# violetdenim/c3dgs

Measured on AMD Instinct MI355X. Metric: raster views/sec fwd+bwd @1920x1080, higher is better.
Workload: dtype f32; 1 GPU; BASELINE.json configs[2]: synth-v1 3M Gaussians, SH deg 3, indexed-camera rasterizer (QAT inner loop), mark_visible+fwd+bwd, 1 view/step/GPU; gaussians=3000000, width=1920, height=1080, sh_codebook=304096, gaussian_codebook=754096, parallelism=replicas x1

## Files before the change

### c3dgs_amd/build.py

```python
import os
import subprocess
import sys
from concurrent.futures import ThreadPoolExecutor

HERE = os.path.dirname(os.path.abspath(__file__))
CSRC = os.path.join(HERE, "csrc")
OBJ = os.path.join(HERE, "build")
LIB = os.path.join(HERE, "libc3dgs_hip.so")
HIPCC = os.environ.get("HIPCC", "/opt/rocm/bin/hipcc")
ARCH = "gfx950"

COMMON = ["--offload-arch=" + ARCH, "-O3", "-fPIC", "-std=c++17", "-Wall", "-Wno-unused-function",
          "-fno-gpu-rdc", "-DNDEBUG"]
SOURCES = {
    "c_abi.hip": [],
    "c_abi_debug.hip": [],
    "preprocess.hip": ["-ffp-contract=off"],
    "backward_preprocess.hip": ["-ffp-contract=off"] + os.environ.get("C3DGS_BWDPRE_FLAGS", "").split(),
    "binning.hip": [],
    "radix_sort.hip": os.environ.get("C3DGS_SORT_FLAGS", "").split(),
    "render.hip": os.environ.get("C3DGS_RENDER_FLAGS", "-fno-slp-vectorize").split(),
    "render_depth.hip": os.environ.get("C3DGS_RENDER_FLAGS", "-fno-slp-vectorize").split(),
    "vq.hip": ["-mllvm", "-amdgpu-mfma-vgpr-form"] + os.environ.get("C3DGS_VQ_FLAGS", "").split(),
    "draws.hip": [],
    "loss.hip": [],
    "metrics.hip": [],
    "encode.hip": [],
    "knn.hip": ["-ffp-contract=off"],
    "adam.hip": ["-ffp-contract=off"],
    "qat.hip": ["-ffp-contract=off"],
    "densify.hip": ["-ffp-contract=off"],
    "index_plan.hip": [],
    "ray_fill.hip": ["-ffp-contract=off"],
    "image_io.hip": ["-ffp-contract=off"],
}
HEADERS = [os.path.join(CSRC, "common.hpp"), os.path.join(CSRC, "gsmath.hpp"), os.path.join(CSRC, "render_diag.hpp"),
           os.path.join(CSRC, "render_common.hpp"),
           os.path.join(HERE, "..", "include", "c3dgs_hip.h"), os.path.join(HERE, "..", "include", "c3dgs_hip_debug.h")]


def _stale(target, deps):
    if not os.path.exists(target):
        return True
    t = os.path.getmtime(target)
    return any(os.path.getmtime(d) > t for d in deps)


def _compile(name, extra, verbose):
    src = os.path.join(CSRC, name)
    obj = os.path.join(OBJ, name.replace(".hip", ".o"))
    cmd = [HIPCC] + COMMON + extra + ["-c", src, "-o", obj]
    if verbose:
        print(" ".join(cmd), flush=True)
    subprocess.check_call(cmd)
    return obj


VARIANTS = {"spin1": {"radix_sort.hip": ["-DC3DGS_OS_SPIN_LIMIT=1u"]}}
def _diag(mode):
    return {src: ["-DC3DGS_DIAG", mode] for src in ("render.hip", "radix_sort.hip", "diag.hip")}


DIAG_VARIANTS = {"lanes": _diag("-DC3DGS_COUNT_LANES"), "bwdtime": _diag("-DC3DGS_BWD_TIMING"), "ostime": _diag("-DC3DGS_OS_TIMING")}


def build_variant(name, verbose=False):
    build(verbose=verbose)
    flags = {**VARIANTS, **DIAG_VARIANTS}[name]
    odir = os.path.join(HERE, "build", "variant_" + name)
    os.makedirs(odir, exist_ok=True)
    lib = os.path.join(HERE, f"libc3dgs_hip_{name}.so")
    objs, rebuilt = [], False
    for src in list(SOURCES) + [f for f in flags if f not in SOURCES]:
        extra = SOURCES.get(src, [])
        obj = os.path.join(OBJ, src.replace(".hip", ".o"))
        if src in flags:
            obj = os.path.join(odir, src.replace(".hip", ".o"))
            if _stale(obj, [os.path.join(CSRC, src)] + HEADERS + [os.path.abspath(__file__)]):
                cmd = [HIPCC] + COMMON + extra + flags[src] + ["-c", os.path.join(CSRC, src), "-o", obj]
                if verbose:
                    print(" ".join(cmd), flush=True)
                subprocess.check_call(cmd)
                rebuilt = True
        objs.append(obj)
    if rebuilt or _stale(lib, objs):
        subprocess.check_call([HIPCC, "--offload-arch=" + ARCH, "-shared", "-fPIC", "-o", lib] + objs)
    return lib


def build(force=False, verbose=False):
    os.makedirs(OBJ, exist_ok=True)
    deps_common = HEADERS + [os.path.abspath(__file__)]
    todo, objs = [], []
    for name, extra in SOURCES.items():
        obj = os.path.join(OBJ, name.replace(".hip", ".o"))
        objs.append(obj)
        if force or _stale(obj, [os.path.join(CSRC, name)] + deps_common):
            todo.append((name, extra))
    if todo:
        with ThreadPoolExecutor(max_workers=min(4, len(todo))) as ex:
            list(ex.map(lambda t: _compile(t[0], t[1], verbose), todo))
    if force or todo or _stale(LIB, objs):
        cmd = [HIPCC, "--offload-arch=" + ARCH, "-shared", "-fPIC", "-o", LIB] + objs
        if verbose:
            print(" ".join(cmd), flush=True)
        subprocess.check_call(cmd)
    return LIB


if __name__ == "__main__":
    print(build(force="--force" in sys.argv, verbose="--verbose" in sys.argv or "-v" in sys.argv))
    for flag, table in (("--variants", VARIANTS), ("--diag", DIAG_VARIANTS)):
        for v in table if flag in sys.argv else ():
            print(build_variant(v, verbose="--verbose" in sys.argv or "-v" in sys.argv))
```

### c3dgs_amd/csrc/binning.hip

```cpp
#include "common.hpp"
#include <rocprim/device/device_radix_sort.hpp>
#include <rocprim/iterator/counting_iterator.hpp>

namespace c3dgs {

size_t scan_temp_bytes(int P)
{
    size_t a = 0, b = 0;
    (void)rocprim::radix_sort_pairs(nullptr, b, (const uint32_t*)nullptr, (uint32_t*)nullptr, (const uint32_t*)nullptr,
                                    (uint32_t*)nullptr, (size_t)P, 0u, 32u);
    size_t m = a > b ? a : b;
    const size_t os = onesweep_depth_temp_bytes(P);
    if (os > m) m = os;
    return m < 256 ? 256 : m;
}

size_t sort_temp_bytes(int R, int end_bit, int key_bytes)
{
    size_t bytes = 0;
    if (key_bytes == 4)
        (void)rocprim::radix_sort_pairs(nullptr, bytes, (const uint32_t*)nullptr, (uint32_t*)nullptr,
                                        (const uint32_t*)nullptr, (uint32_t*)nullptr, (size_t)R, 0u, (unsigned)end_bit);
    else
        (void)rocprim::radix_sort_pairs(nullptr, bytes, (const uint16_t*)nullptr, (uint16_t*)nullptr,
                                        (const uint32_t*)nullptr, (uint32_t*)nullptr, (size_t)R, 0u, (unsigned)end_bit);
    const size_t os = onesweep_tile_temp_bytes(R, end_bit, key_bytes);
    if (os > bytes) bytes = os;
    const size_t reuse = compact_bin_layout(R).bin_bytes;
    if (reuse > bytes) bytes = reuse;
    return bytes < 256 ? 256 : bytes;
}

__global__ void __launch_bounds__(256)
gather_u64_kernel(int n, const uint32_t* __restrict__ idx, const uint2* __restrict__ src, uint2* __restrict__ dst)
{
    const int i = blockIdx.x * 256 + threadIdx.x;
    if (i < n) dst[i] = src[idx[i]];
}

size_t depth_sort_clear_bytes(int P)
{
    return (onesweep_enabled() && (size_t)P < ((size_t)1 << 30)) ? onesweep_depth_clear_bytes(P) : 0;
}
size_t tile_sort_clear_bytes(int R, int end_bit, int key_bytes)
{
    return (onesweep_enabled() && (size_t)R < ((size_t)1 << 30)) ? onesweep_tile_clear_bytes(R, end_bit, key_bytes) : 0;
}

hipError_t run_depth_sort(void* temp, size_t temp_bytes, const uint32_t* kin, uint32_t* kout, const uint32_t* vin,
                          uint32_t* vout, int P, const uint2* rects, uint2* rects_sorted, hipStream_t s, bool ctrl_cleared,
                          bool rects_fit_bytes)
{
    if (onesweep_enabled() && (size_t)P < ((size_t)1 << 30))
        return onesweep_depth_sort(temp, temp_bytes, kin, kout, vin, vout, P, rects, rects_sorted, s, ctrl_cleared, rects_fit_bytes);
    hipError_t e = vin ? rocprim::radix_sort_pairs(temp, temp_bytes, kin, kout, vin, vout, (size_t)P, 0u, 32u, s)
                       : rocprim::radix_sort_pairs(temp, temp_bytes, kin, kout, rocprim::counting_iterator<uint32_t>(0u), vout,
                                                   (size_t)P, 0u, 32u, s);
    if (e != hipSuccess) return e;
    gather_u64_kernel<<<(P + 255) / 256, 256, 0, s>>>(P, vout, rects, rects_sorted);
    return hipGetLastError();
}

hipError_t run_tile_sort(void* temp, size_t temp_bytes, const void* kin, void* kout, int key_bytes, const uint32_t* vin,
                         uint32_t* vout, int R, int end_bit, hipStream_t s, bool ctrl_cleared)
{
    if (key_bytes == 4) {
        if (onesweep_enabled() && (size_t)R < ((size_t)1 << 30))
            return onesweep_tile_sort32(temp, temp_bytes, (const uint32_t*)kin, (uint32_t*)kout, vin, vout, R, end_bit, s, ctrl_cleared);
        return rocprim::radix_sort_pairs(temp, temp_bytes, (const uint32_t*)kin, (uint32_t*)kout, vin, vout, (size_t)R, 0u, (unsigned)end_bit, s);
    }
    if (onesweep_enabled() && (size_t)R < ((size_t)1 << 30))
        return onesweep_tile_sort(temp, temp_bytes, (const uint16_t*)kin, (uint16_t*)kout, vin, vout, R, end_bit, s, ctrl_cleared);
    return rocprim::radix_sort_pairs(temp, temp_bytes, (const uint16_t*)kin, (uint16_t*)kout, vin, vout, (size_t)R, 0u, (unsigned)end_bit, s);
}

}
```

### c3dgs_amd/csrc/c_abi.hip

```cpp
#include "common.hpp"
#include <cfloat>
#include <climits>
#include <cstdlib>
#include <cstring>
#include <mutex>
#include <vector>

namespace c3dgs {

static thread_local std::string g_last_error;
void set_error(const std::string& msg) { g_last_error = msg; }

#define C3DGS_STAGE_TABLE(X)                                                                                                   \
    X(MARK_VISIBLE, "mark_visible") X(PREPROCESS, "preprocess") X(DEPTH_SORT, "depth_sort") X(SCAN, "scan")                    \
    X(DUPLICATE, "duplicate_with_keys") X(SORT, "sort") X(RANGES, "identify_ranges") X(RENDER_FWD, "render_forward")           \
    X(RENDER_DEPTH, "render_depth")                                                                                            \
    X(ZERO_PARTIALS, "zero_partials") X(RENDER_BWD, "render_backward") X(BWD_PREPROCESS, "backward_preprocess")                \
    X(WDIST, "weighted_distance") X(VQ_ACC, "vq_accumulate") X(VQ_APPLY, "vq_apply") X(LOSS_FWD, "l1_ssim_forward")            \
    X(LOSS_BWD, "l1_ssim_backward") X(QAT_OBSERVE, "qat_observe") X(QAT_CODEBOOKS, "qat_codebooks")                            \
    X(QAT_VISIBLE, "qat_visible") X(QAT_POINTS, "qat_points") X(QAT_POINTS_BWD, "qat_points_backward")                         \
    X(QAT_CODEBOOKS_BWD, "qat_codebooks_backward") X(ADAM, "adam_step") X(KNN_SORT, "knn_sort") X(KNN_BOUNDS, "knn_bounds")    \
    X(KNN_QUERY, "knn_query")
#define C3DGS_X(id, name) ST_##id,
enum Stage { C3DGS_STAGE_TABLE(C3DGS_X) ST_COUNT };
#undef C3DGS_X
#define C3DGS_X(id, name) name,
static const char* const kStageNames[ST_COUNT] = { C3DGS_STAGE_TABLE(C3DGS_X) };
#undef C3DGS_X
struct ProfRec { int stage; hipEvent_t a, b; };
static std::mutex g_prof_mu;
static bool g_prof_on = false;
static int g_prof_only = -1;
static std::vector<ProfRec> g_prof_recs;
static std::vector<hipEvent_t> g_prof_pool;

struct StageTimer {
    bool on; int stage; hipStream_t s; hipEvent_t a{}, b{};
    StageTimer(int stage_, hipStream_t s_) : on(g_prof_on && (g_prof_only < 0 || g_prof_only == stage_)), stage(stage_), s(s_)
    {
        if (!on) return;
        std::lock_guard<std::mutex> lk(g_prof_mu);
        auto get = [&](hipEvent_t& e) {
            if (!g_prof_pool.empty()) { e = g_prof_pool.back(); g_prof_pool.pop_back(); }
            else if (hipEventCreate(&e) != hipSuccess) on = false;
        };
        get(a); get(b);
        if (on) (void)hipEventRecord(a, s);
    }
    ~StageTimer()
    {
        if (!on) return;
        (void)hipEventRecord(b, s);
        std::lock_guard<std::mutex> lk(g_prof_mu);
        g_prof_recs.push_back({ stage, a, b });
    }
};
#define C3DGS_STAGE_CHECK(stage, debug, stream) C3DGS_STAGE(kStageNames[stage], debug, stream)
#define C3DGS_TIMED_STAGE(stage, debug, stream, ...)                                                \
    do {                                                                                            \
        { StageTimer t_(stage, stream); __VA_ARGS__; }                                              \
        C3DGS_STAGE_CHECK(stage, debug, stream);                                                    \
    } while (0)

struct HostRead {
    uint32_t* pinned = nullptr;
    uint32_t* dev = nullptr;
    uint32_t seq = 0;
    hipEvent_t ev{};
    HostRead()
    {
        const char* e = std::getenv("C3DGS_HOST_READ_COPY");
        const bool want_map = !(e && e[0] == '1');
        if (want_map && hipHostMalloc((void**)&pinned, 64, hipHostMallocMapped | hipHostMallocPortable | hipHostMallocCoherent) == hipSuccess) {
            void* d = nullptr;
            if (hipHostGetDevicePointer(&d, pinned, 0) == hipSuccess) dev = (uint32_t*)d;
            std::memset(pinned, 0, 64);
        } else {
            (void)hipGetLastError();
            if (hipHostMalloc((void**)&pinned, 64, hipHostMallocDefault) != hipSuccess) { pinned = nullptr; return; }
        }
        if (hipEventCreateWithFlags(&ev, hipEventDisableTiming) != hipSuccess) { (void)hipHostFree(pinned); pinned = nullptr; dev = nullptr; }
    }
    uint32_t begin()
    {
        if (!dev) return 0u;
        if (++seq == 0u) seq = 1u;
        return seq;
    }
    int copy_words(const uint32_t* src, hipStream_t s)
    {
        C3DGS_HIP_TRY(hipMemcpyAsync(pinned, src, 2 * sizeof(uint32_t), hipMemcpyDeviceToHost, s));
        return C3DGS_OK;
    }
    int queue_copy(const uint32_t* src, hipStream_t s)
    {
        if (dev) return C3DGS_OK;
        if (int rc = copy_words(src, s)) return rc;
        C3DGS_HIP_TRY(hipEventRecord(ev, s));
        return C3DGS_OK;
    }
    int wait(const uint32_t* src, hipStream_t s, uint32_t words[2])
    {
        if (dev) {
            volatile uint32_t* pad = pinned;
            bool seen = false;
            for (long spins = 0; !seen; spins++) {
                seen = __atomic_load_n(&pad[2], __ATOMIC_ACQUIRE) == seq;
                if (!seen && (spins & 0xffff) == 0xffff) {
                    const hipError_t q = hipStreamQuery(s);
                    if (q == hipErrorNotReady) continue;
                    if (q != hipSuccess) return fail(C3DGS_E_HIP, std::string("num_rendered read: ") + hipGetErrorString(q));
                    seen = __atomic_load_n(&pad[2], __ATOMIC_ACQUIRE) == seq;
                    if (!seen) {
                        if (int rc = copy_words(src, s)) return rc;
                        C3DGS_HIP_TRY(hipStreamSynchronize(s));
                        seen = true;
                    }
                }
            }
        } else {
            hipError_t q = hipErrorNotReady;
            for (long spins = 0; spins < 20000000L && (q = hipEventQuery(ev)) == hipErrorNotReady; spins++) { }
            if (q == hipErrorNotReady) q = hipEventSynchronize(ev);
            if (q != hipSuccess) return fail(C3DGS_E_HIP, std::string("num_rendered read: ") + hipGetErrorString(q));
        }
        words[0] = pinned[0]; words[1] = pinned[1];
        return C3DGS_OK;
    }
};
static HostRead& host_read()
{
    static thread_local HostRead h;
    return h;
}

static int validate(const c3dgs_raster_params* p, bool indexed, bool is_backward)
{
    if (!p) return fail(C3DGS_E_INVALID, "params is NULL");
    if (p->P < 0 || p->W <= 0 || p->H <= 0) return fail(C3DGS_E_INVALID, "P, W, H must be non-negative / positive");
    if (p->P == 0) return C3DGS_OK;
    if (!p->means3D) return fail(C3DGS_E_INVALID, "means3D must have dimensions (num_points, 3)");
    if (!p->background || !p->viewmatrix || !p->projmatrix || !p->campos)
        return fail(C3DGS_E_INVALID, "background, viewmatrix, projmatrix and campos are required");
    if (!is_backward && !p->opacities)
        return fail(C3DGS_E_INVALID, "opacities is required");
    if ((p->sh == nullptr) == (p->colors_precomp == nullptr))
        return fail(C3DGS_E_INVALID, "Please provide excatly one of either SHs or precomputed colors!");
    const bool has_sr = p->scales != nullptr && p->rotations != nullptr;
    if ((p->scales != nullptr) != (p->rotations != nullptr) || has_sr == (p->cov3D_precomp != nullptr))
        return fail(C3DGS_E_INVALID, "Please provide exactly one of either scale/rotation pair or precomputed 3D covariance!");
    if (p->sh) {
        if (p->D < 0 || p->D > 3) return fail(C3DGS_E_INVALID, "SH degree must be in [0,3]");
        if (p->M < (p->D + 1) * (p->D + 1)) return fail(C3DGS_E_INVALID, "sh has fewer coefficients than the active degree needs");
    }
    if (indexed) {
        if (p->sh && !p->sh_indices) return fail(C3DGS_E_INVALID, "indexed rasterizer: sh_indices is required with sh");
        if (has_sr && (!p->g_indices || !p->scale_factors))
            return fail(C3DGS_E_INVALID, "indexed rasterizer: g_indices and scale_factors are required with scales/rotations");
    } else if (p->sh_indices || p->g_indices || p->scale_factors) {
        return fail(C3DGS_E_INVALID, "non-indexed rasterizer: sh_indices / g_indices / scale_factors must be NULL");
    }
    if (tiles_x(p->W) > 65535 || tiles_y(p->H) > 65535) return fail(C3DGS_E_INVALID, "image too large for 16-bit tile coordinates");
    if ((unsigned long long)tiles_x(p->W) * tiles_x(p->W) * tiles_y(p->H) >= (1ull << 32))
        return fail(C3DGS_E_INVALID, "image too large: (tiles per row)^2 x (tile rows) must stay below 2^32");
    return C3DGS_OK;
}

static int forward_impl(const c3dgs_raster_params* pp, bool indexed, c3dgs_resize_fn geom_resize, void* geom_user,
                        c3dgs_resize_fn binning_resize, void* binning_user, c3dgs_resize_fn image_resize, void* image_user,
                        float* out_color, int32_t* radii, int32_t* num_rendered, void* stream_)
{
    if (int rc = validate(pp, indexed, false)) return rc;
    if (!out_color || !num_rendered) return fail(C3DGS_E_INVALID, "out_color and num_rendered are required");
    if (!geom_resize || !binning_resize || !image_resize) return fail(C3DGS_E_INVALID, "resize callbacks are required");
    c3dgs_raster_params p = *pp;
    if (!indexed) { p.sh_indices = nullptr; p.g_indices = nullptr; p.scale_factors = nullptr; }
    hipStream_t s = (hipStream_t)stream_;
    const int P = p.P, W = p.W, H = p.H;
    const int gx = tiles_x(W), gy = tiles_y(H);
    *num_rendered = 0;

    ImageLayout IL; image_layout(W, H, &IL);
    void* img_base = image_resize(image_user, IL.total_bytes);
    if (!img_base) return fail(C3DGS_E_ALLOC, "image buffer allocation failed");
    const ImgPtrs img = img_ptrs(img_base, W, H);

    if (P == 0) {
        C3DGS_HIP_TRY(hipMemsetAsync(out_color, 0, (size_t)3 * W * H * sizeof(float), s));
        C3DGS_HIP_TRY(hipMemsetAsync(img_base, 0, IL.total_bytes, s));
        return C3DGS_OK;
    }
    if (!radii) return fail(C3DGS_E_INVALID, "radii is required");

    c3dgs_geom_layout GL; geom_layout(P, &GL);
    void* geom_base = geom_resize(geom_user, GL.total_bytes + geom_gtab_bytes(p));
    if (!geom_base) return fail(C3DGS_E_ALLOC, "geometry buffer allocation failed");
    const GeomPtrs g = geom_ptrs(geom_base, P);

    uint32_t* sort_err = onesweep_error_word();
    if (!sort_err) return fail(C3DGS_E_HIP, "cannot resolve the sort error word");
    HostRead& hr = host_read();
    if (!hr.pinned) return fail(C3DGS_E_HIP, "pinned host buffer allocation failed");
    const uint32_t host_seq = hr.begin();
    const size_t dclear = depth_sort_clear_bytes(P) <= g.scan_temp_bytes ? depth_sort_clear_bytes(P) : 0;
    { StageTimer t_(ST_PREPROCESS, s);
      if (geom_gtab_bytes(p)) launch_pack_codebook(p, g.gtab, s);
      launch_preprocess(p, g, radii, img.ranges, sort_err, g.scan_temp, dclear / 16, hr.dev, host_seq, s); }
    C3DGS_STAGE_CHECK(ST_PREPROCESS, p.debug, s);
    const uint32_t* r_words = g.block_base + (P + 255) / 256;
    if (int rc = hr.queue_copy(r_words, s)) return rc;
    { StageTimer t_(ST_DEPTH_SORT, s);
      C3DGS_HIP_TRY(run_depth_sort(g.scan_temp, g.scan_temp_bytes, g.depth_keys, g.depth_keys_sorted, nullptr, g.depth_order, P,
                                   reinterpret_cast<const uint2*>(g.rects), g.sorted_offsets, s, dclear != 0,
                                   gx <= 255 && gy <= 255)); }
    C3DGS_STAGE_CHECK(ST_DEPTH_SORT, p.debug, s);
    if (p.debug && onesweep_timed_out(s)) return fail(C3DGS_E_HIP, "depth sort: look-back timed out");
    C3DGS_TIMED_STAGE(ST_SCAN, p.debug, s, launch_depth_order_scan(P, g, s));
    uint32_t words[2];
    if (int rc = hr.wait(r_words, s, words)) return rc;
    const uint32_t R_u = words[0];
    if (words[1] != 0) {
        C3DGS_HIP_TRY(hipMemsetAsync(sort_err, 0, sizeof(uint32_t), s));
        return fail(C3DGS_E_HIP, "radix sort look-back timed out in an earlier rasterizer call on this device: that call's "
                                 "image is NaN and its gradients are invalid (flag cleared, this call was not run)");
    }
    if (R_u > 0x7fffffffu) return fail(C3DGS_E_INVALID, "num_rendered overflows int32");
    const int R = (int)R_u;
    *num_rendered = R;

    c3dgs_binning_layout BL; binning_layout(R, W, H, &BL);
    void* bin_base = binning_resize(binning_user, BL.total_bytes);
    if (!bin_base) return fail(C3DGS_E_ALLOC, "binning buffer allocation failed");
    const BinPtrs b = bin_ptrs(bin_base, R, W, H);

    if (R > 0) {
        const int end_bit = tile_sort_end_bit(W, H);
        size_t tclear = tile_sort_clear_bytes(R, end_bit, b.key_bytes);
        if (tclear > b.sort_temp_bytes) tclear = 0;
        C3DGS_TIMED_STAGE(ST_DUPLICATE, p.debug, s, launch_duplicate_with_keys(P, g, b, gx, sort_err, b.sort_temp, tclear / 16, s));
        { StageTimer t_(ST_SORT, s);
          C3DGS_HIP_TRY(run_tile_sort(b.sort_temp, b.sort_temp_bytes, b.keys_unsorted, b.keys_sorted, b.key_bytes, b.values_unsorted,
                                      b.point_list, R, end_bit, s, tclear != 0)); }
        C3DGS_STAGE_CHECK(ST_SORT, p.debug, s);
        if (p.debug && onesweep_timed_out(s)) return fail(C3DGS_E_HIP, "tile sort: look-back timed out");
        C3DGS_TIMED_STAGE(ST_RANGES, p.debug, s, launch_identify_ranges(R, b.keys_sorted, b.key_bytes, img.ranges, sort_err, s));
    }
    C3DGS_TIMED_STAGE(ST_RENDER_FWD, p.debug, s,
                      launch_render_forward(W, H, img, b.point_list, g.splat, p.background, out_color, compact_ptrs(b, R), sort_err, s));
    return C3DGS_OK;
}

static int backward_impl(const c3dgs_raster_params* pp, bool indexed, const int32_t* radii, const void* geom_buffer,
                         const void* binning_buffer, const void* image_buffer, int32_t R, const float* dL_dout_color,
                         c3dgs_resize_fn ws_resize, void* ws_user, const c3dgs_raster_grads* grads, void* stream_)
{
    if (int rc = validate(pp, indexed, true)) return rc;
    if (!grads) return fail(C3DGS_E_INVALID, "grads is NULL");
    c3dgs_raster_params p = *pp;
    if (!indexed) { p.sh_indices = nullptr; p.g_indices = nullptr; p.scale_factors = nullptr; }
    hipStream_t s = (hipStream_t)stream_;
    const int P = p.P, W = p.W, H = p.H;

    void* cb_zero = nullptr;
    size_t cb_zero16 = 0;
    if (indexed) {
        const size_t n_sh = (grads->dL_dsh && p.sh) ? (size_t)p.SHS * p.M * 3 * sizeof(float) : 0;
        const size_t n_rot = (grads->dL_drotations && p.scales) ? (size_t)p.GS * 4 * sizeof(float) : 0;
        const size_t n_sc = (grads->dL_dscales && p.scales) ? (size_t)p.GS * 3 * sizeof(float) : 0;
        char* a_sh = (char*)grads->dL_dsh; char* a_rot = (char*)grads->dL_drotations; char* a_sc = (char*)grads->dL_dscales;
        if (n_sh && n_rot && n_sc && a_rot == a_sh + n_sh && a_sc == a_rot + n_rot) {
            const size_t n = n_sh + n_rot + n_sc;
            if (p.P > 0 && R >= 0 && ((uintptr_t)a_sh & 15u) == 0) {
                cb_zero = a_sh; cb_zero16 = n / 16;
                if (n % 16) C3DGS_HIP_TRY(hipMemsetAsync(a_sh + cb_zero16 * 16, 0, n % 16, s));
            } else {
                C3DGS_HIP_TRY(hipMemsetAsync(a_sh, 0, n, s));
            }
        } else {
            if (n_sh) C3DGS_HIP_TRY(hipMemsetAsync(a_sh, 0, n_sh, s));
            if (n_sc) C3DGS_HIP_TRY(hipMemsetAsync(a_sc, 0, n_sc, s));
            if (n_rot) C3DGS_HIP_TRY(hipMemsetAsync(a_rot, 0, n_rot, s));
        }
    }
    if (P == 0) return C3DGS_OK;
    if (!radii || !geom_buffer || !image_buffer || !dL_dout_color || (R > 0 && !binning_buffer))
        return fail(C3DGS_E_INVALID, "radii, forward buffers and dL_dout_color are required");
    if (!ws_resize) return fail(C3DGS_E_INVALID, "workspace callback is required");
    if (R < 0) return fail(C3DGS_E_INVALID, "R must be >= 0");

    const GeomPtrs g = geom_ptrs(const_cast<void*>(geom_buffer), P);
    const ImgPtrs img = img_ptrs(const_cast<void*>(image_buffer), W, H);
    void* ws_base = ws_resize(ws_user, c3dgs_backward_workspace_bytes(P, R));
    if (!ws_base) return fail(C3DGS_E_ALLOC, "backward workspace allocation failed");
    const BwdPtrs w = bwd_ptrs(ws_base, P, R);

    { StageTimer t_(ST_ZERO_PARTIALS, s);
      launch_backward_prep(R > 0 ? W : 0, H, img, w.touched, w.touched_bytes / 16, R > 0 ? nullptr : cb_zero, R > 0 ? 0 : cb_zero16, s); }
    if (R > 0) {
        const BinPtrs b = bin_ptrs(const_cast<void*>(binning_buffer), R, W, H);
        C3DGS_TIMED_STAGE(ST_RENDER_BWD, p.debug, s,
                          launch_render_backward(W, H, img, g.splat, g.block_base, p.background, dL_dout_color, w.partials, w.touched,
                                                 compact_ptrs(b, R), cb_zero, cb_zero16, s));
    }
    C3DGS_TIMED_STAGE(ST_BWD_PREPROCESS, p.debug, s, launch_backward_preprocess(p, radii, g, w, *grads, s));
    return C3DGS_OK;
}

}

using namespace c3dgs;

extern "C" {

const char* c3dgs_last_error(void) { return g_last_error.c_str(); }

int c3dgs_profile_enable(int on)
{
    std::lock_guard<std::mutex> lk(g_prof_mu);
    g_prof_on = on != 0;
    return C3DGS_OK;
}

int c3dgs_profile_only(const char* stage_name)
{
    std::lock_guard<std::mutex> lk(g_prof_mu);
    g_prof_only = -1;
    if (!stage_name || !*stage_name) return C3DGS_OK;
    for (int i = 0; i < ST_COUNT; i++)
        if (std::strcmp(stage_name, kStageNames[i]) == 0) { g_prof_only = i; return C3DGS_OK; }
    return fail(C3DGS_E_INVALID, std::string("profile_only: unknown stage ") + stage_name);
}

int c3dgs_profile_read(c3dgs_stage_time* out, int capacity)
{
    std::vector<ProfRec> recs;
    {
        std::lock_guard<std::mutex> lk(g_prof_mu);
        recs.swap(g_prof_recs);
    }
    double total[ST_COUNT] = { 0 };
    long long count[ST_COUNT] = { 0 };
    for (auto& r : recs) {
        float ms = 0.f;
        if (hipEventSynchronize(r.b) == hipSuccess && hipEventElapsedTime(&ms, r.a, r.b) == hipSuccess) {
            total[r.stage] += (double)ms;
            count[r.stage]++;
        }
    }
    {
        std::lock_guard<std::mutex> lk(g_prof_mu);
        for (auto& r : recs) { g_prof_pool.push_back(r.a); g_prof_pool.push_back(r.b); }
    }
    int n = 0;
    for (int i = 0; i < ST_COUNT && n < capacity; i++) {
        if (!count[i]) continue;
        std::memset(&out[n], 0, sizeof(out[n]));
        std::strncpy(out[n].name, kStageNames[i], sizeof(out[n].name) - 1);
        out[n].total_ms = total[i];
        out[n].count = count[i];
        n++;
    }
    return n;
}
int c3dgs_abi_version(void) { return C3DGS_ABI_VERSION; }

int c3dgs_get_geom_layout(int32_t P, c3dgs_geom_layout* out)
{
    if (!out || P < 0) return fail(C3DGS_E_INVALID, "bad arguments");
    geom_layout(P, out);
    return C3DGS_OK;
}
int c3dgs_get_binning_layout(int32_t R, int32_t W, int32_t H, c3dgs_binning_layout* out)
{
    if (!out || R < 0 || W <= 0 || H <= 0) return fail(C3DGS_E_INVALID, "bad arguments");
    binning_layout(R, W, H, out);
    return C3DGS_OK;
}
int c3dgs_get_image_layout(int32_t W, int32_t H, c3dgs_image_layout* out)
{
    if (!out || W <= 0 || H <= 0) return fail(C3DGS_E_INVALID, "bad arguments");
    ImageLayout L; image_layout(W, H, &L);
    *out = L;
    return C3DGS_OK;
}
int c3dgs_get_compact_layout(int32_t R, int32_t W, int32_t H, c3dgs_compact_layout* out)
{
    if (!out || R < 0 || W <= 0 || H <= 0) return fail(C3DGS_E_INVALID, "bad arguments");
    c3dgs_binning_layout BL; binning_layout(R, W, H, &BL);
    const CompactBinLayout C = compact_bin_layout(R);
    ImageLayout IL; image_layout(W, H, &IL);
    out->cqm = BL.sort_temp + C.cqm; out->cid = BL.sort_temp + C.cid;
    out->tile_used_c = IL.tile_used_c; out->n_contrib_c = IL.n_contrib_c;
    return C3DGS_OK;
}
int c3dgs_get_backward_layout(int32_t P, int32_t R, c3dgs_backward_layout* out)
{
    if (!out || P < 0 || R < 0) return fail(C3DGS_E_INVALID, "bad arguments");
    backward_layout(P, R, out);
    return C3DGS_OK;
}
size_t c3dgs_backward_workspace_bytes(int32_t P, int32_t R)
{
    c3dgs_backward_layout L; backward_layout(P, R, &L);
    return L.total_bytes;
}

int c3dgs_mark_visible(int32_t P, const float* means3D, const float* viewmatrix, const float* projmatrix, uint8_t* present,
                       void* stream)
{
    (void)projmatrix;
    if (P < 0) return fail(C3DGS_E_INVALID, "P must be >= 0");
    if (P == 0) return C3DGS_OK;
    if (!means3D || !viewmatrix || !present) return fail(C3DGS_E_INVALID, "means3D, viewmatrix and present are required");
    C3DGS_TIMED_STAGE(ST_MARK_VISIBLE, 0, (hipStream_t)stream, launch_mark_visible(P, means3D, viewmatrix, present, (hipStream_t)stream));
    return C3DGS_OK;
}

int c3dgs_mark_visible_pose(int32_t P, const float* means3D, const float* extrinsic_vector, uint8_t* present, void* stream)
{
    if (P < 0) return fail(C3DGS_E_INVALID, "P must be >= 0");
    if (P == 0) return C3DGS_OK;
    if (!means3D || !extrinsic_vector || !present) return fail(C3DGS_E_INVALID, "means3D, extrinsic_vector and present are required");
    C3DGS_TIMED_STAGE(ST_MARK_VISIBLE, 0, (hipStream_t)stream, launch_mark_visible_pose(P, means3D, extrinsic_vector, present, (hipStream_t)stream));
    return C3DGS_OK;
}

int c3dgs_camera_from_pose(const float* extrinsic_vector, float inv_tan_half_fovx, float inv_tan_half_fovy, float* viewmatrix,
                           float* projmatrix, float* campos, void* stream)
{
    if (!extrinsic_vector || !viewmatrix || !projmatrix || !campos) return fail(C3DGS_E_INVALID, "camera_from_pose: NULL pointer");
    launch_camera_from_pose(extrinsic_vector, inv_tan_half_fovx, inv_tan_half_fovy, viewmatrix, projmatrix, campos, (hipStream_t)stream);
    C3DGS_STAGE("camera_from_pose", 0, (hipStream_t)stream);
    return C3DGS_OK;
}

int c3dgs_rasterize_gaussians(const c3dgs_raster_params* p, c3dgs_resize_fn geom_resize, void* geom_user,
                              c3dgs_resize_fn binning_resize, void* binning_user, c3dgs_resize_fn image_resize,
                              void* image_user, float* out_color, int32_t* radii, int32_t* num_rendered, void* stream)
{
    return forward_impl(p, false, geom_resize, geom_user, binning_resize, binning_user, image_resize, image_user, out_color,
                        radii, num_rendered, stream);
}

int c3dgs_rasterize_gaussians_indexed(const c3dgs_raster_params* p, c3dgs_resize_fn geom_resize, void* geom_user,
                                      c3dgs_resize_fn binning_resize, void* binning_user, c3dgs_resize_fn image_resize,
                                      void* image_user, float* out_color, int32_t* radii, int32_t* num_rendered, void* stream)
{
    return forward_impl(p, true, geom_resize, geom_user, binning_resize, binning_user, image_resize, image_user, out_color,
                        radii, num_rendered, stream);
}

int c3dgs_rasterize_gaussians_backward(const c3dgs_raster_params* p, const int32_t* radii, const void* geom_buffer,
                                       const void* binning_buffer, const void* image_buffer, int32_t R,
                                       const float* dL_dout_color, c3dgs_resize_fn workspace_resize, void* workspace_user,
                                       const c3dgs_raster_grads* grads, void* stream)
{
    return backward_impl(p, false, radii, geom_buffer, binning_buffer, image_buffer, R, dL_dout_color, workspace_resize,
                         workspace_user, grads, stream);
}

int c3dgs_rasterize_gaussians_backward_indexed(const c3dgs_raster_params* p, const int32_t* radii, const void* geom_buffer,
                                               const void* binning_buffer, const void* image_buffer, int32_t R,
                                               const float* dL_dout_color, c3dgs_resize_fn workspace_resize,
                                               void* workspace_user, const c3dgs_raster_grads* grads, void* stream)
{
    return backward_impl(p, true, radii, geom_buffer, binning_buffer, image_buffer, R, dL_dout_color, workspace_resize,
                         workspace_user, grads, stream);
}

int c3dgs_render_depth(int32_t P, int32_t W, int32_t H, int32_t R, const void* geom_buffer, const void* binning_buffer,
                       const void* image_buffer, float* out_depth, float* out_alpha, float* out_median, void* stream)
{
    if (W <= 0 || H <= 0) return fail(C3DGS_E_INVALID, "render_depth: W and H must be positive");
    if (P < 0 || R < 0) return fail(C3DGS_E_INVALID, "render_depth: P and R must be >= 0");
    if (!out_depth && !out_alpha && !out_median) return fail(C3DGS_E_INVALID, "render_depth: at least one output is required");
    if (R > 0 && P == 0) return fail(C3DGS_E_INVALID, "render_depth: R > 0 instances cannot come from P = 0");
    if (R > 0 && (!geom_buffer || !binning_buffer || !image_buffer))
        return fail(C3DGS_E_INVALID, "render_depth: the forward's geometry, binning and image buffers are required");
    hipStream_t s = (hipStream_t)stream;
    if (P == 0 || R == 0) {
        const size_t bytes = (size_t)W * H * sizeof(float);
        for (float* o : { out_depth, out_alpha, out_median })
            if (o) C3DGS_HIP_TRY(hipMemsetAsync(o, 0, bytes, s));
        return C3DGS_OK;
    }
    uint32_t* sort_err = onesweep_error_word();
    if (!sort_err) return fail(C3DGS_E_HIP, "cannot resolve the sort error word");
    const GeomPtrs g = geom_ptrs(const_cast<void*>(geom_buffer), P);
    const ImgPtrs img = img_ptrs(const_cast<void*>(image_buffer), W, H);
    const BinPtrs b = bin_ptrs(const_cast<void*>(binning_buffer), R, W, H);
    C3DGS_TIMED_STAGE(ST_RENDER_DEPTH, 0, s,
                      launch_render_depth(W, H, img, compact_ptrs(b, R), g.splat, g.depth_keys, out_depth, out_alpha, out_median,
                                          sort_err, s));
    return C3DGS_OK;
}

int c3dgs_weighted_distance(int64_t N, int32_t C, int32_t K, const float* coefs, const int64_t* gather,
                            const float* codebook, float* out_dist, int64_t* out_idx, void* stream)
{
    if (N < 0 || C < 0 || K <= 0) return fail(C3DGS_E_INVALID, "coefs and codebook must have same number of channels");
    if (N == 0) return C3DGS_OK;
    if (!coefs || !codebook || !out_dist || !out_idx) return fail(C3DGS_E_INVALID, "ceofs and codebook must have dimension 2");
    {
        StageTimer t_(ST_WDIST, (hipStream_t)stream);
        if (launch_weighted_distance(N, C, K, coefs, gather, codebook, out_dist, out_idx, (hipStream_t)stream))
            return fail(C3DGS_E_INVALID, "unsupported channel count");
    }
    C3DGS_STAGE_CHECK(ST_WDIST, 0, (hipStream_t)stream);
    return C3DGS_OK;
}

size_t c3dgs_weighted_distance_ws_bytes(int64_t N, int32_t C, int32_t K) { return wd_ws_bytes(N, C, K); }

int c3dgs_weighted_distance_ws(int64_t N, int32_t C, int32_t K, const float* coefs, const int64_t* gather, const float* codebook,
                               float* out_dist, int64_t* out_idx, void* ws, size_t ws_bytes, void* stream)
{
    if (N < 0 || C < 0 || K <= 0) return fail(C3DGS_E_INVALID, "coefs and codebook must have same number of channels");
    if (N == 0) return C3DGS_OK;
    if (!coefs || !codebook || !out_dist || !out_idx) return fail(C3DGS_E_INVALID, "ceofs and codebook must have dimension 2");
    {
        StageTimer t_(ST_WDIST, (hipStream_t)stream);
        if (launch_weighted_distance(N, C, K, coefs, gather, codebook, out_dist, out_idx, (hipStream_t)stream, ws, ws ? ws_bytes : 0))
            return fail(C3DGS_E_INVALID, "unsupported channel count");
    }
    C3DGS_STAGE_CHECK(ST_WDIST, 0, (hipStream_t)stream);
    return C3DGS_OK;
}

int c3dgs_vq_accumulate(int64_t B, int32_t K, int32_t D, const float* x, const float* w, const int64_t* gather,
                        const int64_t* idx, const float* dist, float* S, double* dist_sum, void* stream)
{
    if (B < 0 || K <= 0 || D <= 0) return fail(C3DGS_E_INVALID, "bad sizes");
    if (B == 0) return C3DGS_OK;
    if (!x || !w || !idx || !S) return fail(C3DGS_E_INVALID, "x, w, idx and S are required");
    C3DGS_TIMED_STAGE(ST_VQ_ACC, 0, (hipStream_t)stream, launch_vq_accumulate(B, K, D, x, w, gather, idx, dist, S, dist_sum, (hipStream_t)stream));
    return C3DGS_OK;
}

int c3dgs_vq_sums(int64_t B, int32_t K, int32_t D, const float* x, const float* w, const int64_t* gather,
                  const float* codebook, float* dist, int64_t* idx, float* S, double* dist_sum, void* ws, size_t ws_bytes,
                  void* stream)
{
    if (B < 0 || K <= 0 || D <= 0) return fail(C3DGS_E_INVALID, "bad sizes");
    if (!S || !dist_sum) return fail(C3DGS_E_INVALID, "S and dist_sum are required");
    C3DGS_HIP_TRY(hipMemsetAsync(S, 0, (size_t)K * (D + 1) * sizeof(float), (hipStream_t)stream));
    C3DGS_HIP_TRY(hipMemsetAsync(dist_sum, 0, sizeof(double), (hipStream_t)stream));
    if (B == 0) return C3DGS_OK;
    if (!x || !w || !codebook || !dist || !idx) return fail(C3DGS_E_INVALID, "x, w, codebook, dist and idx are required");
    {
        StageTimer t_(ST_WDIST, (hipStream_t)stream);
        if (launch_weighted_distance(B, K, D, x, gather, codebook, dist, idx, (hipStream_t)stream, ws, ws ? ws_bytes : 0))
            return fail(C3DGS_E_INVALID, "unsupported channel count");
    }
    C3DGS_STAGE_CHECK(ST_WDIST, 0, (hipStream_t)stream);
    return c3dgs_vq_accumulate(B, K, D, x, w, gather, idx, dist, S, dist_sum, stream);
}

int c3dgs_vq_step_supported(int32_t K, int32_t D, const float* x, const float* codebook, const void* ws, size_t ws_bytes)
{
    return (K > 0 && D > 0 && wd_presplit_supported(K, D, x, codebook, ws, ws_bytes)) ? 1 : 0;
}

int c3dgs_vq_step_sums(int32_t step, int64_t B, int32_t K, int32_t D, const float* x, const float* w, const int64_t* gather,
                       const float* codebook, float* dist, int64_t* idx, float* S, double* dist_sum, void* ws, size_t ws_bytes,
                       void* stream)
{
    hipStream_t s = (hipStream_t)stream;
    if (step < 0 || B <= 0 || K <= 0 || D <= 0) return fail(C3DGS_E_INVALID, "vq_step_sums: bad sizes");
    if (!x || !w || !codebook || !dist || !idx || !S || !dist_sum) return fail(C3DGS_E_INVALID, "vq_step_sums: NULL argument");
    if (!wd_presplit_supported(K, D, x, codebook, ws, ws_bytes))
        return fail(C3DGS_E_INVALID, "vq_step_sums: shape / scratch not served by the fused step (see c3dgs_vq_step_supported)");
    if (step == 0) {
        C3DGS_HIP_TRY(hipMemsetAsync(S, 0, (size_t)K * (D + 1) * sizeof(float), s));
        C3DGS_HIP_TRY(hipMemsetAsync(dist_sum, 0, sizeof(double), s));
    }
    {
        StageTimer t_(ST_WDIST, s);
        if (launch_weighted_distance(B, K, D, x, gather, codebook, dist, idx, s, ws, ws_bytes, step == 0 ? -1 : (step & 1)))
            return fail(C3DGS_E_INVALID, "vq_step_sums: unsupported shape");
        if (step == 0) launch_vq_seed_words(K, D, ws, s);
    }
    C3DGS_STAGE_CHECK(ST_WDIST, 0, s);
    C3DGS_TIMED_STAGE(ST_VQ_ACC, 0, s,
                      launch_vq_accumulate(B, K, D, x, w, gather, idx, dist, S, dist_sum, s, vq_next_absmax_word(K, D, ws, step & 1)));
    return C3DGS_OK;
}

int c3dgs_vq_step_apply(int32_t step, int32_t K, int32_t D, float* S, float* codebook, float* entry_importance, float decay,
                        float alpha, float eps, int32_t scale_normalize, void* ws, size_t ws_bytes, void* stream)
{
    if (step < 0 || K <= 0 || D <= 0 || !S || !codebook || !entry_importance) return fail(C3DGS_E_INVALID, "vq_step_apply: bad arguments");
    { StageTimer t_(ST_VQ_APPLY, (hipStream_t)stream);
      if (launch_vq_apply_split(K, D, S, codebook, entry_importance, decay, alpha, eps, scale_normalize, ws, ws_bytes, step & 1, (hipStream_t)stream))
          return fail(C3DGS_E_INVALID, "vq_step_apply: shape / scratch not served by the fused step (see c3dgs_vq_step_supported)"); }
    C3DGS_STAGE_CHECK(ST_VQ_APPLY, 0, (hipStream_t)stream);
    return C3DGS_OK;
}

int c3dgs_vq_apply(int32_t K, int32_t D, const float* S, float* codebook, float* entry_importance, float decay,
                   float alpha, float eps, int32_t scale_normalize, void* stream)
{
    if (K <= 0 || D <= 0 || !S || !codebook || !entry_importance) return fail(C3DGS_E_INVALID, "bad arguments");
    C3DGS_TIMED_STAGE(ST_VQ_APPLY, 0, (hipStream_t)stream,
                      launch_vq_apply(K, D, S, codebook, entry_importance, decay, alpha, eps, scale_normalize, (hipStream_t)stream));
    return C3DGS_OK;
}

size_t c3dgs_morton_workspace_bytes(int32_t P) { return morton_workspace_bytes(P); }

int c3dgs_morton_order(int32_t P, const float* xyz, int64_t* codes, int64_t* order, void* workspace, void* stream)
{
    if (P < 0) return fail(C3DGS_E_INVALID, "P must be >= 0");
    if (P == 0) return C3DGS_OK;
    if (!xyz || !codes || !order || !workspace) return fail(C3DGS_E_INVALID, "morton_order: bad arguments");
    if (run_morton_order(P, xyz, codes, order, workspace, (hipStream_t)stream)) return fail(C3DGS_E_HIP, "morton_order failed");
    C3DGS_STAGE("morton_order", 0, (hipStream_t)stream);
    return C3DGS_OK;
}

size_t c3dgs_knn_workspace_bytes(int32_t P) { return knn_workspace_bytes(P); }

int c3dgs_knn_mean_dist2(int32_t P, const float* xyz, float* out, void* workspace, void* stream)
{
    if (P < 0) return fail(C3DGS_E_INVALID, "knn_mean_dist2: P must be >= 0");
    if (P == 0) return C3DGS_OK;
    if (!xyz || !out || !workspace) return fail(C3DGS_E_INVALID, "knn_mean_dist2: bad arguments");
    hipStream_t s = (hipStream_t)stream;
    { StageTimer t_(ST_KNN_SORT, s);
      if (run_knn_sort(P, xyz, workspace, s)) return fail(C3DGS_E_HIP, "knn_mean_dist2: sort failed"); }
    C3DGS_STAGE_CHECK(ST_KNN_SORT, 0, s);
    C3DGS_TIMED_STAGE(ST_KNN_BOUNDS, 0, s, launch_knn_bounds(P, workspace, s));
    C3DGS_TIMED_STAGE(ST_KNN_QUERY, 0, s, launch_knn_query(P, workspace, out, s));
    return C3DGS_OK;
}

int c3dgs_knn_neighbours(int32_t P, const float* xyz, int32_t* idx, float* d2, void* workspace, void* stream)
{
    if (P < 0) return fail(C3DGS_E_INVALID, "knn_neighbours: P must be >= 0");
    if (P == 0) return C3DGS_OK;
    if (!xyz || !idx || !d2 || !workspace) return fail(C3DGS_E_INVALID, "knn_neighbours: bad arguments");
    hipStream_t s = (hipStream_t)stream;
    { StageTimer t_(ST_KNN_SORT, s);
      if (run_knn_sort(P, xyz, workspace, s)) return fail(C3DGS_E_HIP, "knn_neighbours: sort failed"); }
    C3DGS_STAGE_CHECK(ST_KNN_SORT, 0, s);
    C3DGS_TIMED_STAGE(ST_KNN_BOUNDS, 0, s, launch_knn_bounds(P, workspace, s));
    C3DGS_TIMED_STAGE(ST_KNN_QUERY, 0, s, launch_knn_query_neighbours(P, workspace, idx, d2, s));
    return C3DGS_OK;
}

int c3dgs_abs_accumulate(int64_t n, const float* g, float* acc, void* stream)
{
    if (n < 0 || (n > 0 && (!g || !acc))) return fail(C3DGS_E_INVALID, "abs_accumulate: bad arguments");
    launch_abs_accumulate(n, g, acc, (hipStream_t)stream);
    C3DGS_STAGE("abs_accumulate", 0, (hipStream_t)stream);
    return C3DGS_OK;
}

int c3dgs_adam_step(int32_t n_tensors, const c3dgs_adam_tensor* tensors, double beta1, double beta2, double eps, void* stream)
{
    if (n_tensors < 0 || n_tensors > C3DGS_ADAM_MAX_TENSORS) return fail(C3DGS_E_INVALID, "adam_step: between 0 and 16 tensors per call");
    if (n_tensors == 0) return C3DGS_OK;
    if (!tensors) return fail(C3DGS_E_INVALID, "adam_step: tensors is NULL");
    for (int k = 0; k < n_tensors; k++)
        if (tensors[k].n > 0 && (!tensors[k].param || !tensors[k].grad || !tensors[k].exp_avg || !tensors[k].exp_avg_sq))
            return fail(C3DGS_E_INVALID, "adam_step: NULL tensor pointer");
    C3DGS_TIMED_STAGE(ST_ADAM, 0, (hipStream_t)stream, launch_adam(n_tensors, tensors, beta1, beta2, eps, (hipStream_t)stream));
    return C3DGS_OK;
}

static const int kRowsMaxCopies = 250;

int c3dgs_densify_classify(int32_t P, const float* accum, const float* denom, const float* scale_clone, const float* scale_split,
                           const float* scale_prune_self, const float* scale_prune_child, const float* opacity, float max_grad,
                           float dense_extent, float min_opacity, float big_extent, uint8_t* code, void* stream)
{
    if (P < 0) return fail(C3DGS_E_INVALID, "densify_classify: P must be >= 0");
    if (!(max_grad > 0.f)) return fail(C3DGS_E_INVALID, "densify_classify: max_grad must be > 0 (see include/c3dgs_hip.h)");
    if (P == 0) return C3DGS_OK;
    if (!accum || !denom || !scale_clone || !scale_split || !opacity || !code)
        return fail(C3DGS_E_INVALID, "densify_classify: NULL buffer");
    if ((scale_prune_self == nullptr) != (scale_prune_child == nullptr))
        return fail(C3DGS_E_INVALID, "densify_classify: scale_prune_self and scale_prune_child go together");
    launch_densify_classify(P, accum, denom, scale_clone, scale_split, scale_prune_self, scale_prune_child, opacity, max_grad,
                            dense_extent, min_opacity, big_extent, code, (hipStream_t)stream);
    C3DGS_STAGE("densify_classify", 0, (hipStream_t)stream);
    return C3DGS_OK;
}

size_t c3dgs_rows_plan_workspace_bytes(int32_t P) { return rows_plan_workspace_bytes(P); }

int c3dgs_rows_plan(int32_t P, const uint8_t* code, int32_t N, int64_t capacity, int32_t* src, uint8_t* kind, int32_t* draw_row,
                    int32_t* totals, void* workspace, void* stream)
{
    if (P < 0) return fail(C3DGS_E_INVALID, "rows_plan: P must be >= 0");
    if (N < 1 || N > kRowsMaxCopies) return fail(C3DGS_E_INVALID, "rows_plan: N must be between 1 and 250");
    if (capacity < 0) return fail(C3DGS_E_INVALID, "rows_plan: capacity must be >= 0");
    if ((int64_t)P * (2 + N) >= ((int64_t)1 << 31)) return fail(C3DGS_E_INVALID, "rows_plan: P * (2 + N) must fit 31 bits");
    if (!totals) return fail(C3DGS_E_INVALID, "rows_plan: totals is required");
    hipStream_t s = (hipStream_t)stream;
    if (P == 0) { C3DGS_HIP_TRY(hipMemsetAsync(totals, 0, 4 * sizeof(int32_t), s)); return C3DGS_OK; }
    if (!code || !workspace) return fail(C3DGS_E_INVALID, "rows_plan: NULL buffer");
    if (src && (!kind || !draw_row)) return fail(C3DGS_E_INVALID, "rows_plan: src, kind and draw_row go together");
    C3DGS_HIP_TRY(run_rows_plan(P, code, N, capacity, src, kind, draw_row, totals, workspace, s));
    C3DGS_STAGE("rows_plan", 0, s);
    return C3DGS_OK;
}

int c3dgs_rows_apply(int32_t P, int64_t P_new, const int32_t* src, const uint8_t* kind, const int32_t* draw_row, int32_t n_tensors,
                     const c3dgs_rows_tensor* tensors, int32_t N, int64_t n_draws, const float* rotation_raw, const float* std,
                     const float* z, int32_t log_scaling, int32_t half_xyz, void* stream)
{
    if (P < 0 || P_new < 0 || n_draws < 0) return fail(C3DGS_E_INVALID, "rows_apply: sizes must be >= 0");
    if (N < 1 || N > kRowsMaxCopies) return fail(C3DGS_E_INVALID, "rows_apply: N must be between 1 and 250");
    if (n_tensors < 0 || n_tensors > C3DGS_ROWS_MAX_TENSORS) return fail(C3DGS_E_INVALID, "rows_apply: between 0 and 16 tensors per call");
    if (P_new >= ((int64_t)1 << 31)) return fail(C3DGS_E_INVALID, "rows_apply: P_new must fit 31 bits");
    if (P_new == 0 || n_tensors == 0) return C3DGS_OK;
    if (P == 0) return fail(C3DGS_E_INVALID, "rows_apply: P_new > 0 rows cannot come from P = 0");
    if (!src || !kind || !draw_row || !tensors) return fail(C3DGS_E_INVALID, "rows_apply: NULL buffer");
    for (int k = 0; k < n_tensors; k++) {
        const c3dgs_rows_tensor& t = tensors[k];
        if (t.row_floats < 1 || t.row_floats > 4096) return fail(C3DGS_E_INVALID, "rows_apply: row_floats must be between 1 and 4096");
        if (!t.in_param || !t.out_param) return fail(C3DGS_E_INVALID, "rows_apply: NULL tensor pointer");
        const int nm = (t.in_exp_avg != nullptr) + (t.in_exp_avg_sq != nullptr) + (t.out_exp_avg != nullptr) + (t.out_exp_avg_sq != nullptr);
        if (nm != 0 && nm != 4) return fail(C3DGS_E_INVALID, "rows_apply: the four moment pointers go together");
        if (t.role != C3DGS_ROLE_COPY && t.role != C3DGS_ROLE_XYZ && t.role != C3DGS_ROLE_SCALING)
            return fail(C3DGS_E_INVALID, "rows_apply: unknown role");
        if (t.role != C3DGS_ROLE_COPY && t.row_floats != 3) return fail(C3DGS_E_INVALID, "rows_apply: xyz / scaling rows have 3 floats");
        if (t.role != C3DGS_ROLE_COPY && n_draws > 0 && (!std || !z || (t.role == C3DGS_ROLE_XYZ && !rotation_raw)))
            return fail(C3DGS_E_INVALID, "rows_apply: children need rotation_raw, std and z");
    }
    launch_rows_apply(P, P_new, src, kind, draw_row, n_tensors, tensors, N, n_draws, rotation_raw, std, z, log_scaling, half_xyz, (hipStream_t)stream);
    C3DGS_STAGE("rows_apply", 0, (hipStream_t)stream);
    return C3DGS_OK;
}

int c3dgs_densify_stats(int32_t P, const float* grad, const uint8_t* filter, const int32_t* radii, float* accum, float* denom,
                        float* max_radii, void* stream)
{
    if (P < 0) return fail(C3DGS_E_INVALID, "densify_stats: P must be >= 0");
    if (P == 0) return C3DGS_OK;
    if (!grad || !filter || !accum || !denom) return fail(C3DGS_E_INVALID, "densify_stats: NULL buffer");
    if ((radii == nullptr) != (max_radii == nullptr)) return fail(C3DGS_E_INVALID, "densify_stats: radii and max_radii go together");
    launch_densify_stats(P, grad, filter, radii, accum, denom, max_radii, (hipStream_t)stream);
    C3DGS_STAGE("densify_stats", 0, (hipStream_t)stream);
    return C3DGS_OK;
}

size_t c3dgs_ray_fill_plan_workspace_bytes(int32_t P, int64_t rows) { return ray_fill_plan_workspace_bytes(P, rows); }

int c3dgs_ray_fill_plan(int32_t P, const float* d2, float step, int64_t capacity, int32_t* src, uint8_t* slot, int32_t* level,
                        int32_t* totals, void* workspace, size_t workspace_bytes, void* stream)
{
    if (P < 0 || capacity < 0) return fail(C3DGS_E_INVALID, "ray_fill_plan: P and capacity must be >= 0");
    if (P > INT32_MAX - 255) return fail(C3DGS_E_INVALID, "ray_fill_plan: P must be at most INT32_MAX - 255");
    if (!(step > 0.f) || !(step <= FLT_MAX)) return fail(C3DGS_E_INVALID, "ray_fill_plan: step must be a positive finite number");
    if (!totals) return fail(C3DGS_E_INVALID, "ray_fill_plan: totals is required");
    if (src && (!slot || !level)) return fail(C3DGS_E_INVALID, "ray_fill_plan: src, slot and level go together");
    hipStream_t s = (hipStream_t)stream;
    if (P == 0) { C3DGS_HIP_TRY(hipMemsetAsync(totals, 0, 4 * sizeof(int32_t), s)); return C3DGS_OK; }
    if (!d2 || !workspace) return fail(C3DGS_E_INVALID, "ray_fill_plan: NULL buffer");
    std::string problem;
    C3DGS_HIP_TRY(run_ray_fill_plan(P, d2, step, capacity, src, slot, level, totals, workspace, workspace_bytes, s, &problem));
    if (!problem.empty()) return fail(C3DGS_E_INVALID, "ray_fill_plan: " + problem);
    C3DGS_STAGE("ray_fill_plan", 0, s);
    return C3DGS_OK;
}

int c3dgs_ray_fill_xyz(int32_t P, const float* xyz, const int32_t* idx, const float* d2, float step, int64_t n_new,
                       const int32_t* src, const uint8_t* slot, const int32_t* level, float* out, void* stream)
{
    if (P < 0 || n_new < 0) return fail(C3DGS_E_INVALID, "ray_fill_xyz: sizes must be >= 0");
    if (n_new > INT32_MAX - 255) return fail(C3DGS_E_INVALID, "ray_fill_xyz: n_new must be at most INT32_MAX - 255");
    if (!(step > 0.f) || !(step <= FLT_MAX)) return fail(C3DGS_E_INVALID, "ray_fill_xyz: step must be a positive finite number");
    if (n_new == 0) return C3DGS_OK;
    if (!xyz || !idx || !d2 || !src || !slot || !level || !out) return fail(C3DGS_E_INVALID, "ray_fill_xyz: NULL buffer");
    launch_ray_fill_xyz(P, xyz, idx, d2, step, n_new, src, slot, level, out, (hipStream_t)stream);
    C3DGS_STAGE("ray_fill_xyz", 0, (hipStream_t)stream);
    return C3DGS_OK;
}

int c3dgs_image_from_u8(int32_t Hs, int32_t Ws, int32_t C, const uint8_t* src, int32_t flip, const float* bg, int32_t Hd, int32_t Wd,
                        float* out, void* stream)
{
    const int32_t kMax = 32768;
    if (Hs < 1 || Ws < 1 || Hd < 1 || Wd < 1 || Hs > kMax || Ws > kMax || Hd > kMax || Wd > kMax)
        return fail(C3DGS_E_INVALID, "image_from_u8: every dimension must be in [1, 32768]");
    if (C != 3 && C != 4) return fail(C3DGS_E_INVALID, "image_from_u8: C must be 3 or 4");
    if (bg && C == 3) return fail(C3DGS_E_INVALID, "image_from_u8: a background needs an alpha channel (C == 4)");
    if (!src || !out) return fail(C3DGS_E_INVALID, "image_from_u8: NULL buffer");
    launch_image_from_u8(Hs, Ws, C, src, flip != 0, bg, Hd, Wd, out, (hipStream_t)stream);
    C3DGS_STAGE("image_from_u8", 0, (hipStream_t)stream);
    return C3DGS_OK;
}

static const int32_t kIndexPlanMaxRows = INT32_MAX - 255;

size_t c3dgs_index_plan_workspace_bytes(int32_t P, int32_t K0, int32_t K1) { return index_plan_workspace_bytes(P, K0, K1); }

int c3dgs_index_plan(int32_t P, const uint8_t* keep, const int64_t* idx0, int32_t K0, const int64_t* idx1, int32_t K1, int64_t cap_rows,
                     int64_t cap_cb0, int64_t cap_cb1, int32_t* src, int64_t* new_idx0, int64_t* new_idx1, int32_t* cb_src0,
                     int32_t* cb_src1, int32_t* totals, void* workspace, void* stream)
{
    if (P < 0 || K0 < 0 || K1 < 0) return fail(C3DGS_E_INVALID, "index_plan: P, K0 and K1 must be >= 0");
    if (P > kIndexPlanMaxRows || K0 > kIndexPlanMaxRows || K1 > kIndexPlanMaxRows)
        return fail(C3DGS_E_INVALID, "index_plan: P, K0 and K1 must be at most INT32_MAX - 255");
    if (cap_rows < 0 || cap_cb0 < 0 || cap_cb1 < 0) return fail(C3DGS_E_INVALID, "index_plan: capacities must be >= 0");
    if ((idx0 && K0 <= 0) || (idx1 && K1 <= 0)) return fail(C3DGS_E_INVALID, "index_plan: an index array needs a codebook of K > 0 rows");
    if (!totals) return fail(C3DGS_E_INVALID, "index_plan: totals is required");
    if (!workspace) return fail(C3DGS_E_INVALID, "index_plan: workspace is required");
    if (src && ((idx0 && (!new_idx0 || !cb_src0)) || (idx1 && (!new_idx1 || !cb_src1))))
        return fail(C3DGS_E_INVALID, "index_plan: src, and new_idx and cb_src of every index space given, go together");
    hipStream_t s = (hipStream_t)stream;
    if (P == 0) { C3DGS_HIP_TRY(hipMemsetAsync(totals, 0, 4 * sizeof(int32_t), s)); return C3DGS_OK; }
    C3DGS_HIP_TRY(run_index_plan(P, keep, idx0, K0, idx1, K1, cap_rows, cap_cb0, cap_cb1, src, new_idx0, new_idx1, cb_src0, cb_src1,
                                 totals, workspace, s));
    C3DGS_STAGE("index_plan", 0, s);
    return C3DGS_OK;
}

int c3dgs_extract_rot_scale(int32_t n, const float* cov6, float* rot, float* scale, void* stream)
{
    if (n < 0) return fail(C3DGS_E_INVALID, "extract_rot_scale: n must be >= 0");
    if (n == 0) return C3DGS_OK;
    if (!cov6 || !rot || !scale || (reinterpret_cast<uintptr_t>(rot) & 15)) return fail(C3DGS_E_INVALID, "extract_rot_scale: bad arguments");
    launch_extract_rot_scale(n, cov6, rot, scale, (hipStream_t)stream);
    C3DGS_STAGE("extract_rot_scale", 0, (hipStream_t)stream);
    return C3DGS_OK;
}

int c3dgs_l1_ssim_forward(int32_t C, int32_t H, int32_t W, const float* img, const float* gt, float* dmaps, double* sums,
                          void* stream)
{
    if (C <= 0 || H <= 0 || W <= 0 || !img || !gt || !sums) return fail(C3DGS_E_INVALID, "l1_ssim_forward: bad arguments");
    hipStream_t s = (hipStream_t)stream;
    C3DGS_HIP_TRY(hipMemsetAsync(sums, 0, 128 * sizeof(double), s));
    const size_t n = (size_t)C * H * W;
    C3DGS_TIMED_STAGE(ST_LOSS_FWD, 0, s,
                      launch_l1_ssim_forward(C, H, W, img, gt, dmaps, dmaps ? dmaps + n : nullptr, dmaps ? dmaps + 2 * n : nullptr, sums, s));
    return C3DGS_OK;
}

int c3dgs_l1_ssim_value(const double* sums, double l1_scale, double ssim_scale, double constant, float* out, void* stream)
{
    if (!sums || !out) return fail(C3DGS_E_INVALID, "l1_ssim_value: bad arguments");
    launch_l1_ssim_value(sums, l1_scale, ssim_scale, constant, out, (hipStream_t)stream);
    C3DGS_STAGE("l1_ssim_value", 0, (hipStream_t)stream);
    return C3DGS_OK;
}

int c3dgs_l1_ssim_backward(int32_t C, int32_t H, int32_t W, const float* img, const float* gt, const float* dmaps,
                           const float* grad_loss, float l1_coeff, float ssim_coeff, float* dL_dimg, void* stream)
{
    if (C <= 0 || H <= 0 || W <= 0 || !img || !gt || !dmaps || !grad_loss || !dL_dimg)
        return fail(C3DGS_E_INVALID, "l1_ssim_backward: bad arguments");
    hipStream_t s = (hipStream_t)stream;
    const size_t n = (size_t)C * H * W;
    C3DGS_TIMED_STAGE(ST_LOSS_BWD, 0, s,
                      launch_l1_ssim_backward(C, H, W, img, gt, dmaps, dmaps + n, dmaps + 2 * n, grad_loss, l1_coeff, ssim_coeff, dL_dimg, s));
    return C3DGS_OK;
}

size_t c3dgs_image_metrics_ws_bytes(int32_t N, int32_t C, int32_t H, int32_t W) { return image_metrics_ws_bytes(N, C, H, W); }

int c3dgs_image_metrics(int32_t N, int32_t C, int32_t H, int32_t W, const float* img, const float* gt, void* ws, size_t ws_bytes,
                        double* out, void* stream)
{
    if (N <= 0 || C <= 0 || H <= 0 || W <= 0) return fail(C3DGS_E_INVALID, "image_metrics: N, C, H and W must be positive");
    if (image_metrics_workgroups(N, C, H, W) > IMAGE_METRICS_MAX_WORKGROUPS)
        return fail(C3DGS_E_INVALID, "image_metrics: size overflow (N * C * H * W too large for one call; split the batch)");
    if (!img || !gt || !ws || !out) return fail(C3DGS_E_INVALID, "image_metrics: img, gt, ws and out are required");
    if (reinterpret_cast<uintptr_t>(ws) & 7) return fail(C3DGS_E_INVALID, "image_metrics: ws must be 8-byte aligned");
    const size_t need = image_metrics_ws_bytes(N, C, H, W);
    if (ws_bytes < need)
        return fail(C3DGS_E_INVALID, "image_metrics: ws too small (" + std::to_string(ws_bytes) + " bytes, need " +
                                         std::to_string(need) + ")");
    launch_image_metrics(N, C, H, W, img, gt, (double*)ws, out, (hipStream_t)stream);
    C3DGS_STAGE("image_metrics", 0, (hipStream_t)stream);
    return C3DGS_OK;
}

static int qat_validate(const c3dgs_qat_params* q, const char* who)
{
    if (!q) return fail(C3DGS_E_INVALID, std::string(who) + ": params is NULL");
    if (q->P < 0 || q->GS < 0 || q->SHS < 0 || q->M < 1) return fail(C3DGS_E_INVALID, std::string(who) + ": bad sizes");
    if (!q->state) return fail(C3DGS_E_INVALID, std::string(who) + ": state is required");
    if (q->features_dc && q->M > 1 && !q->features_rest)
        return fail(C3DGS_E_INVALID, std::string(who) + ": features_rest is required with features_dc when M > 1");
    if (reinterpret_cast<uintptr_t>(q->rotation) & 15) return fail(C3DGS_E_INVALID, std::string(who) + ": rotation must be 16-byte aligned");
    return C3DGS_OK;
}
static bool misaligned16(const void* p) { return (reinterpret_cast<uintptr_t>(p) & 15) != 0; }

size_t c3dgs_qat_workspace_bytes(void) { return qat_workspace_bytes(); }
size_t c3dgs_qat_scan_bytes(int32_t P) { return qat_scan_bytes(P); }

int c3dgs_qat_observe(const c3dgs_qat_params* q, void* workspace, void* stream)
{
    if (int rc = qat_validate(q, "qat_observe")) return rc;
    if (!workspace) return fail(C3DGS_E_INVALID, "qat_observe: workspace is required");
    C3DGS_TIMED_STAGE(ST_QAT_OBSERVE, 0, (hipStream_t)stream, launch_qat_observe(*q, workspace, (hipStream_t)stream));
    return C3DGS_OK;
}

int c3dgs_qat_codebooks(const c3dgs_qat_params* q, float* scales_n, float* rotations, float* shs, void* stream)
{
    if (int rc = qat_validate(q, "qat_codebooks")) return rc;
    if (misaligned16(rotations) || misaligned16(shs)) return fail(C3DGS_E_INVALID, "qat_codebooks: outputs must be 16-byte aligned");
    C3DGS_TIMED_STAGE(ST_QAT_CODEBOOKS, 0, (hipStream_t)stream, launch_qat_codebooks(*q, scales_n, rotations, shs, (hipStream_t)stream));
    return C3DGS_OK;
}

int c3dgs_qat_codebooks_backward(const c3dgs_qat_params* q, const float* dL_dscales_n, const float* dL_drotations,
                                 const float* dL_dshs, float* dL_dscaling, float* dL_drotation, float* dL_dfeatures_dc,
                                 float* dL_dfeatures_rest, void* stream)
{
    if (int rc = qat_validate(q, "qat_codebooks_backward")) return rc;
    if (misaligned16(dL_drotations) || misaligned16(dL_drotation) || misaligned16(dL_dshs))
        return fail(C3DGS_E_INVALID, "qat_codebooks_backward: rotation / sh gradients must be 16-byte aligned");
    if (dL_dshs && q->features_dc && (!dL_dfeatures_dc || (q->M > 1 && !dL_dfeatures_rest)))
        return fail(C3DGS_E_INVALID, "qat_codebooks_backward: dL_dfeatures_dc / dL_dfeatures_rest are required with dL_dshs");
    C3DGS_TIMED_STAGE(ST_QAT_CODEBOOKS_BWD, 0, (hipStream_t)stream,
                      launch_qat_codebooks_backward(*q, dL_dscales_n, dL_drotations, dL_dshs, dL_dscaling, dL_drotation, dL_dfeatures_dc,
                                                    dL_dfeatures_rest, (hipStream_t)stream));
    return C3DGS_OK;
}

int c3dgs_qat_visible(const c3dgs_qat_params* q, const float* viewmatrix, uint8_t* visible, int32_t* rank, int32_t* count,
                      void* scan_workspace, void* stream)
{
    if (int rc = qat_validate(q, "qat_visible")) return rc;
    if (!count) return fail(C3DGS_E_INVALID, "qat_visible: count is required");
    hipStream_t s = (hipStream_t)stream;
    if (q->P == 0) { C3DGS_HIP_TRY(hipMemsetAsync(count, 0, sizeof(int32_t), s)); return C3DGS_OK; }
    if (!q->xyz || !viewmatrix || !visible || !rank || !scan_workspace) return fail(C3DGS_E_INVALID, "qat_visible: bad arguments");
    { StageTimer t_(ST_QAT_VISIBLE, s); C3DGS_HIP_TRY(run_qat_visible(*q, viewmatrix, visible, rank, count, scan_workspace, s)); }
    C3DGS_STAGE_CHECK(ST_QAT_VISIBLE, 0, s);
    return C3DGS_OK;
}

int c3dgs_qat_points(const c3dgs_qat_params* q, const uint8_t* visible, const int32_t* rank, const int64_t* sh_indices,
                     const int64_t* g_indices, float* means3D, float* opacities, float* scale_factors, int64_t* sh_indices_out,
                     int64_t* g_indices_out, void* stream)
{
    if (int rc = qat_validate(q, "qat_points")) return rc;
    if ((visible == nullptr) != (rank == nullptr)) return fail(C3DGS_E_INVALID, "qat_points: visible and rank go together");
    C3DGS_TIMED_STAGE(ST_QAT_POINTS, 0, (hipStream_t)stream,
                      launch_qat_points(*q, visible, rank, sh_indices, g_indices, means3D, opacities, scale_factors, sh_indices_out,
                                        g_indices_out, (hipStream_t)stream));
    return C3DGS_OK;
}

int c3dgs_qat_points_backward(const c3dgs_qat_params* q, const uint8_t* visible, const int32_t* rank, const float* dL_dmeans3D,
                              const float* dL_dmeans2D, const float* dL_dopacities, const float* dL_dscale_factors,
                              float* dL_dxyz, float* dL_dscreenspace, float* dL_dopacity, float* dL_dscaling_factor, void* stream)
{
    if (int rc = qat_validate(q, "qat_points_backward")) return rc;
    if ((visible == nullptr) != (rank == nullptr)) return fail(C3DGS_E_INVALID, "qat_points_backward: visible and rank go together");
    if ((dL_dopacity && dL_dopacities && !q->opacity) || (dL_dscaling_factor && dL_dscale_factors && !q->scaling_factor))
        return fail(C3DGS_E_INVALID, "qat_points_backward: the raw opacity / scaling_factor are needed to recompute the masks");
    C3DGS_TIMED_STAGE(ST_QAT_POINTS_BWD, 0, (hipStream_t)stream,
                      launch_qat_points_backward(*q, visible, rank, dL_dmeans3D, dL_dmeans2D, dL_dopacities, dL_dscale_factors, dL_dxyz,
                                                 dL_dscreenspace, dL_dopacity, dL_dscaling_factor, (hipStream_t)stream));
    return C3DGS_OK;
}

int c3dgs_qat_quantize(const c3dgs_qat_params* q, int32_t scaling_is_exp, int8_t* opacity, int8_t* scaling, int8_t* scaling_factor,
                       int8_t* rotation, int8_t* features_dc, int8_t* features_rest, void* stream)
{
    if (int rc = qat_validate(q, "qat_quantize")) return rc;
    if (rotation && (reinterpret_cast<uintptr_t>(rotation) & 3)) return fail(C3DGS_E_INVALID, "qat_quantize: rotation output must be 4-byte aligned");
    launch_qat_quantize(*q, scaling_is_exp, opacity, scaling, scaling_factor, rotation, features_dc, features_rest, (hipStream_t)stream);
    C3DGS_STAGE("qat_quantize", 0, (hipStream_t)stream);
    return C3DGS_OK;
}

int c3dgs_fake_quantize(int64_t n, const float* x, c3dgs_fq_state* state, int32_t observe, int32_t enabled,
                        float averaging_constant, float* out, void* workspace, void* stream)
{
    if (n < 0) return fail(C3DGS_E_INVALID, "fake_quantize: n must be >= 0");
    if (n == 0) return C3DGS_OK;
    if (!x || !state || !out || (observe && !workspace)) return fail(C3DGS_E_INVALID, "fake_quantize: bad arguments");
    launch_fake_quantize(n, x, state, observe, enabled, averaging_constant, out, workspace, (hipStream_t)stream);
    C3DGS_STAGE("fake_quantize", 0, (hipStream_t)stream);
    return C3DGS_OK;
}

int c3dgs_fake_quantize_backward(int64_t n, const float* x, const c3dgs_fq_state* state, int32_t enabled, const float* g,
                                 float* dx, void* stream)
{
    if (n < 0) return fail(C3DGS_E_INVALID, "fake_quantize_backward: n must be >= 0");
    if (n == 0) return C3DGS_OK;
    if (!x || !state || !g || !dx) return fail(C3DGS_E_INVALID, "fake_quantize_backward: bad arguments");
    launch_fake_quantize_backward(n, x, state, enabled, g, dx, (hipStream_t)stream);
    C3DGS_STAGE("fake_quantize_backward", 0, (hipStream_t)stream);
    return C3DGS_OK;
}

}
```

### c3dgs_amd/csrc/common.hpp

```cpp
#pragma once
#include <hip/hip_runtime.h>
#include <cstdint>
#include <cstddef>
#include <cstdio>
#include <cstring>
#include <string>

#include "../../include/c3dgs_hip.h"

namespace c3dgs {

constexpr int TILE = 16;
constexpr int TILE_PIX = 256;
constexpr int SPLAT_F4 = 3;
constexpr int PARTIAL_FLOATS = 9;
constexpr int BWD_LIST = 1024;

void set_error(const std::string& msg);
inline int fail(int code, const std::string& msg) { set_error(msg); return code; }

#define C3DGS_HIP_TRY(expr)                                                                         \
    do {                                                                                            \
        hipError_t e__ = (expr);                                                                    \
        if (e__ != hipSuccess)                                                                      \
            return ::c3dgs::fail(C3DGS_E_HIP, std::string(#expr) + ": " + hipGetErrorString(e__));  \
    } while (0)

#define C3DGS_STAGE(name, debug, stream)                                                            \
    do {                                                                                            \
        hipError_t e__ = hipGetLastError();                                                         \
        if (e__ == hipSuccess && (debug)) e__ = hipStreamSynchronize(stream);                       \
        if (e__ != hipSuccess)                                                                      \
            return ::c3dgs::fail(C3DGS_E_HIP, std::string("stage ") + name + ": " + hipGetErrorString(e__)); \
    } while (0)

__device__ __forceinline__ uint32_t f2ord(float f)
{
    const uint32_t u = __float_as_uint(f);
    return (u & 0x80000000u) ? ~u : (u | 0x80000000u);
}
__device__ __host__ __forceinline__ float ord2f(uint32_t o)
{
    const uint32_t u = (o & 0x80000000u) ? (o & 0x7fffffffu) : ~o;
    float f;
    memcpy(&f, &u, 4);
    return f;
}

inline size_t align_up(size_t v, size_t a = 256) { return (v + a - 1) / a * a; }

size_t scan_temp_bytes(int P);
size_t sort_temp_bytes(int R, int end_bit, int key_bytes = 2);

inline int tiles_x(int W) { return (W + TILE - 1) / TILE; }
inline int tiles_y(int H) { return (H + TILE - 1) / TILE; }

inline uint32_t higher_msb(uint32_t n)
{
    uint32_t msb = sizeof(n) * 4, step = msb;
    while (step > 1) {
        step /= 2;
        if (n >> msb) msb += step; else msb -= step;
    }
    if (n >> msb) msb++;
    return msb;
}

inline void geom_layout(int P, c3dgs_geom_layout* L)
{
    size_t o = 0, p = (size_t)(P > 0 ? P : 1);
    L->splat = o;             o = align_up(o + p * SPLAT_F4 * 16);
    L->depth_keys = o;        o = align_up(o + p * 4);
    L->depth_keys_sorted = o; o = align_up(o + p * 4);
    L->depth_order = o;       o = align_up(o + p * 4);
    L->sorted_offsets = o;    o = align_up(o + p * 8);
    L->inst_offset = o;       o = align_up(o + p * 4);
    L->rects = o;             o = align_up(o + p * 8);
    L->clamped = o;           o = align_up(o + p);
    L->block_base = o;        o = align_up(o + ((p + 255) / 256 + 2) * 4);
    L->depth_base = o;        o = align_up(o + ((p + 255) / 256 + 1) * 4);
    L->scan_temp = o;         L->scan_temp_bytes = scan_temp_bytes((int)p);
    o = align_up(o + L->scan_temp_bytes);
    L->total_bytes = o;
}

inline size_t geom_gtab_bytes(const c3dgs_raster_params& p) { return (p.g_indices && p.scales) ? align_up((size_t)(p.GS > 0 ? p.GS : 1) * 32) : 0; }

inline int tile_key_bytes_for(long long T) { return T > 65536 ? 4 : 2; }
inline int tile_key_bytes(int W, int H) { return tile_key_bytes_for((long long)tiles_x(W) * tiles_y(H)); }
inline int tile_sort_end_bit_for(long long T)
{
    const int msb = (int)higher_msb((uint32_t)T), kbits = 8 * tile_key_bytes_for(T);
    return msb < kbits ? msb : kbits;
}
inline int tile_sort_end_bit(int W, int H) { return tile_sort_end_bit_for((long long)tiles_x(W) * tiles_y(H)); }

inline void binning_layout(int R, int W, int H, c3dgs_binning_layout* L)
{
    size_t o = 0, r = (size_t)(R > 0 ? R : 1);
    const int end_bit = tile_sort_end_bit(W, H);
    const size_t kb = (size_t)tile_key_bytes(W, H);
    L->keys_unsorted = o;   o = align_up(o + r * kb);
    L->values_unsorted = o; o = align_up(o + r * 4);
    L->keys_sorted = o;     o = align_up(o + r * kb);
    L->point_list = o;      o = align_up(o + r * 4);
    L->sort_temp = o;       L->sort_temp_bytes = sort_temp_bytes((int)r, end_bit, (int)kb);
    o = align_up(o + L->sort_temp_bytes);
    L->total_bytes = o;
}

struct ImageLayout : c3dgs_image_layout { size_t tile_used_c, n_contrib_c; };
inline void image_layout(int W, int H, ImageLayout* L)
{
    size_t o = 0, n = (size_t)W * H, t = (size_t)tiles_x(W) * tiles_y(H);
    L->final_T = o;     o = align_up(o + n * 4);
    L->n_contrib = o;   o = align_up(o + n * 4);
    L->ranges = o;      o = align_up(o + t * 8);
    L->tile_used = o;   o = align_up(o + t * 4);
    L->tile_order = o;  o = align_up(o + t * 4);
    L->tile_used_c = o; o = align_up(o + t * 4);
    L->n_contrib_c = o; o = align_up(o + n * 4);
    L->total_bytes = o;
}

struct CompactBinLayout { size_t cqm, cid, bin_bytes; };
inline CompactBinLayout compact_bin_layout(int R)
{
    const size_t r = (size_t)(R > 0 ? R : 1);
    CompactBinLayout C;
    C.cqm = 0; C.cid = align_up(r); C.bin_bytes = C.cid + align_up(r * 4);
    return C;
}

inline void backward_layout(int P, int R, c3dgs_backward_layout* L)
{
    size_t o = 0, r = (size_t)(R > 0 ? R : 1), n_lists = ((size_t)(P > 0 ? P : 1) + BWD_LIST - 1) / BWD_LIST;
    L->partials = o;   o = align_up(o + r * PARTIAL_FLOATS * sizeof(float));
    L->touched = o;    o = align_up(o + r);
    L->live_ids = o;   o = align_up(o + n_lists * BWD_LIST * 4);
    L->live_slots = o; o = align_up(o + n_lists * BWD_LIST * 4);
    L->live_count = o; o = align_up(o + n_lists * 4);
    L->list_len = BWD_LIST;
    L->total_bytes = o;
}

struct GeomPtrs {
    float4* splat; uint32_t* depth_keys; uint32_t* depth_keys_sorted;
    uint32_t* depth_order; uint2* sorted_offsets; uint32_t* inst_offset; uint16_t* rects;
    uint8_t* clamped; uint32_t* block_base; uint32_t* depth_base; void* scan_temp; size_t scan_temp_bytes;
    float4* gtab;
};
struct BinPtrs {
    void* keys_unsorted; uint32_t* values_unsorted; void* keys_sorted; uint32_t* point_list;
    void* sort_temp; size_t sort_temp_bytes; int key_bytes;
};
struct ImgPtrs { float* final_T; uint32_t* n_contrib; uint2* ranges; uint32_t* tile_used; uint32_t* tile_order;
                 uint32_t* tile_used_c; uint32_t* n_contrib_c; };
struct CompactPtrs { uint8_t* cqm; uint32_t* cid; };
struct BwdPtrs { float* partials; uint8_t* touched; size_t touched_bytes;
                 uint32_t* live_ids; uint32_t* live_slots; uint32_t* live_count; };

inline GeomPtrs geom_ptrs(void* base, int P)
{
    c3dgs_geom_layout L; geom_layout(P, &L);
    char* b = (char*)base;
    return { (float4*)(b + L.splat), (uint32_t*)(b + L.depth_keys), (uint32_t*)(b + L.depth_keys_sorted), (uint32_t*)(b + L.depth_order),
             (uint2*)(b + L.sorted_offsets), (uint32_t*)(b + L.inst_offset), (uint16_t*)(b + L.rects),
             (uint8_t*)(b + L.clamped), (uint32_t*)(b + L.block_base), (uint32_t*)(b + L.depth_base), (void*)(b + L.scan_temp),
             L.scan_temp_bytes, (float4*)(b + L.total_bytes) };
}
inline BinPtrs bin_ptrs(void* base, int R, int W, int H)
{
    c3dgs_binning_layout L; binning_layout(R, W, H, &L);
    char* b = (char*)base;
    return { (void*)(b + L.keys_unsorted), (uint32_t*)(b + L.values_unsorted), (void*)(b + L.keys_sorted),
             (uint32_t*)(b + L.point_list), (void*)(b + L.sort_temp), L.sort_temp_bytes, tile_key_bytes(W, H) };
}
inline ImgPtrs img_ptrs(void* base, int W, int H)
{
    ImageLayout L; image_layout(W, H, &L);
    char* b = (char*)base;
    return { (float*)(b + L.final_T), (uint32_t*)(b + L.n_contrib), (uint2*)(b + L.ranges), (uint32_t*)(b + L.tile_used),
             (uint32_t*)(b + L.tile_order), (uint32_t*)(b + L.tile_used_c), (uint32_t*)(b + L.n_contrib_c) };
}
inline CompactPtrs compact_ptrs(const BinPtrs& bp, int R)
{
    const CompactBinLayout C = compact_bin_layout(R);
    return { (uint8_t*)bp.sort_temp + C.cqm, (uint32_t*)((char*)bp.sort_temp + C.cid) };
}
inline BwdPtrs bwd_ptrs(void* base, int P, int R)
{
    c3dgs_backward_layout L; backward_layout(P, R, &L);
    char* b = (char*)base;
    return { (float*)(b + L.partials), (uint8_t*)(b + L.touched), L.live_ids - L.touched,
             (uint32_t*)(b + L.live_ids), (uint32_t*)(b + L.live_slots), (uint32_t*)(b + L.live_count) };
}

void launch_camera_from_pose(const float* pose, float inv_tan_x, float inv_tan_y, float* view, float* proj, float* campos, hipStream_t s);
void launch_mark_visible(int P, const float* means3D, const float* view, uint8_t* present, hipStream_t s);
void launch_mark_visible_pose(int P, const float* means3D, const float* pose7, uint8_t* present, hipStream_t s);
void launch_pack_codebook(const c3dgs_raster_params& p, float4* gtab, hipStream_t s);
void launch_preprocess(const c3dgs_raster_params& p, const GeomPtrs& g, int32_t* radii, uint2* ranges, const uint32_t* sort_err,
                       void* zero_span, size_t zero_n16, uint32_t* host_out, uint32_t host_seq, hipStream_t s);
void launch_depth_order_scan(int P, const GeomPtrs& g, hipStream_t s);
void launch_duplicate_with_keys(int P, const GeomPtrs& g, const BinPtrs& b, int grid_x, const uint32_t* sort_err,
                                void* zero_span, size_t zero_n16, hipStream_t s);
void launch_identify_ranges(int R, const void* keys_sorted, int key_bytes, uint2* ranges, const uint32_t* sort_err, hipStream_t s);
hipError_t run_depth_sort(void* temp, size_t temp_bytes, const uint32_t* kin, uint32_t* kout, const uint32_t* vin,
                          uint32_t* vout, int P, const uint2* rects, uint2* rects_sorted, hipStream_t s, bool ctrl_cleared = false,
                          bool rects_fit_bytes = false);
hipError_t run_tile_sort(void* temp, size_t temp_bytes, const void* kin, void* kout, int key_bytes, const uint32_t* vin,
                         uint32_t* vout, int R, int end_bit, hipStream_t s, bool ctrl_cleared = false);
size_t depth_sort_clear_bytes(int P);
size_t tile_sort_clear_bytes(int R, int end_bit, int key_bytes);
bool onesweep_enabled();
int onesweep_timed_out(hipStream_t s);
uint32_t* onesweep_error_word();
size_t onesweep_depth_temp_bytes(int P);
size_t onesweep_tile_temp_bytes(int R, int end_bit, int key_bytes = 2);
size_t onesweep_depth_clear_bytes(int P);
size_t onesweep_tile_clear_bytes(int R, int end_bit, int key_bytes);
hipError_t onesweep_depth_sort(void* temp, size_t temp_bytes, const uint32_t* kin, uint32_t* kout, const uint32_t* vin, uint32_t* vout,
                               int P, const uint2* gather_src, uint2* gather_dst, hipStream_t s, bool ctrl_cleared = false,
                               bool rects_fit_bytes = false);
hipError_t onesweep_tile_sort32(void* temp, size_t temp_bytes, const uint32_t* kin, uint32_t* kout, const uint32_t* vin, uint32_t* vout,
                                int R, int end_bit, hipStream_t s, bool ctrl_cleared = false);
hipError_t onesweep_tile_sort(void* temp, size_t temp_bytes, const uint16_t* kin, uint16_t* kout, const uint32_t* vin, uint32_t* vout,
                              int R, int end_bit, hipStream_t s, bool ctrl_cleared = false);
void launch_render_forward(int W, int H, const ImgPtrs& img, const uint32_t* point_list, const float4* splat,
                           const float* bg, float* out_color, const CompactPtrs& cl, const uint32_t* sort_err, hipStream_t s);
void launch_backward_prep(int W, int H, const ImgPtrs& img, void* zero_a, size_t n16_a, void* zero_b, size_t n16_b, hipStream_t s);
void launch_render_backward(int W, int H, const ImgPtrs& img, const float4* splat,
                            const uint32_t* block_base, const float* bg, const float* dL_dpix, float* partials,
                            uint8_t* touched, const CompactPtrs& cl, void* zero_span, size_t zero_n16, hipStream_t s);
void launch_render_depth(int W, int H, const ImgPtrs& img, const CompactPtrs& cl, const float4* splat, const uint32_t* depth_keys,
                         float* out_depth, float* out_alpha, float* out_median, const uint32_t* sort_err, hipStream_t s);
void launch_backward_preprocess(const c3dgs_raster_params& p, const int32_t* radii, const GeomPtrs& g, const BwdPtrs& w,
                                const c3dgs_raster_grads& gr, hipStream_t s);
int launch_weighted_distance(int64_t N, int C, int K, const float* coefs, const int64_t* gather, const float* codebook,
                             float* out_dist, int64_t* out_idx, hipStream_t s, void* ws = nullptr, size_t ws_bytes = 0, int presplit = -1);
bool wd_presplit_supported(int C, int K, const float* coefs, const float* codebook, const void* ws, size_t ws_bytes);
int launch_vq_apply_split(int K, int D, float* S, float* codebook, float* entry_importance, float decay, float alpha, float eps,
                          int scale_normalize, void* ws, size_t ws_bytes, int parity, hipStream_t s);
void launch_vq_seed_words(int K, int D, void* ws, hipStream_t s);
uint32_t* vq_next_absmax_word(int K, int D, void* ws, int parity);
size_t wd_ws_bytes(int64_t N, int C, int K);
int launch_wd_debug_scores(int64_t N, int C, int K, const float* coefs, const float* codebook, float* scores, void* ws, size_t ws_bytes,
                           float* out_dist, int64_t* out_idx, hipStream_t s);
void launch_vq_accumulate(int64_t B, int K, int D, const float* x, const float* w, const int64_t* gather,
                          const int64_t* idx, const float* dist, float* S, double* dist_sum, hipStream_t s, uint32_t* clear_word = nullptr);
void launch_vq_apply(int K, int D, const float* S, float* codebook, float* entry_importance, float decay, float alpha,
                     float eps, int scale_normalize, hipStream_t s);

size_t morton_workspace_bytes(int P);
int run_morton_order(int P, const float* xyz, int64_t* codes_out, int64_t* order_out, void* workspace, hipStream_t s);
void launch_extract_rot_scale(int n, const float* cov6, float* rot, float* scale, hipStream_t s);
size_t knn_workspace_bytes(int P);
int run_knn_sort(int P, const float* xyz, void* workspace, hipStream_t s);
void launch_knn_bounds(int P, void* workspace, hipStream_t s);
void launch_knn_query(int P, const void* workspace, float* out, hipStream_t s);
void launch_knn_query_neighbours(int P, const void* workspace, int32_t* idx, float* d2, hipStream_t s);
size_t ray_fill_plan_workspace_bytes(int P, long long rows);
hipError_t run_ray_fill_plan(int P, const float* d2, float step, long long capacity, int32_t* src, uint8_t* slot, int32_t* level,
                             int32_t* totals, void* workspace, size_t workspace_bytes, hipStream_t s, std::string* problem);
void launch_ray_fill_xyz(int P, const float* xyz, const int32_t* idx, const float* d2, float step, long long n_new,
                         const int32_t* src, const uint8_t* slot, const int32_t* level, float* out, hipStream_t s);
void launch_image_from_u8(int Hs, int Ws, int C, const uint8_t* src, int flip, const float* bg, int Hd, int Wd, float* out,
                          hipStream_t s);
void launch_adam(int n_tensors, const c3dgs_adam_tensor* tensors, double beta1, double beta2, double eps, hipStream_t s);
void launch_abs_accumulate(int64_t n, const float* g, float* acc, hipStream_t s);
void launch_densify_classify(int P, const float* accum, const float* denom, const float* scale_clone, const float* scale_split,
                             const float* scale_prune_self, const float* scale_prune_child, const float* opacity, float max_grad,
                             float dense_extent, float min_opacity, float big_extent, uint8_t* code, hipStream_t s);
size_t rows_plan_workspace_bytes(int P);
hipError_t run_rows_plan(int P, const uint8_t* code, int N, long long capacity, int32_t* src, uint8_t* kind, int32_t* draw_row,
                         int32_t* totals, void* workspace, hipStream_t s);
void launch_rows_apply(int P, long long P_new, const int32_t* src, const uint8_t* kind, const int32_t* draw_row, int n_tensors,
                       const c3dgs_rows_tensor* tensors, int N, long long n_draws, const float* rotation_raw, const float* std,
                       const float* z, int log_scaling, int half_xyz, hipStream_t s);
void launch_densify_stats(int P, const float* grad, const uint8_t* filter, const int32_t* radii, float* accum, float* denom,
                          float* max_radii, hipStream_t s);
size_t index_plan_workspace_bytes(int P, int K0, int K1);
hipError_t run_index_plan(int P, const uint8_t* keep, const int64_t* idx0, int K0, const int64_t* idx1, int K1, long long cap_rows,
                          long long cap_cb0, long long cap_cb1, int32_t* src, int64_t* new_idx0, int64_t* new_idx1, int32_t* cb_src0,
                          int32_t* cb_src1, int32_t* totals, void* workspace, hipStream_t s);
void launch_l1_ssim_value(const double* sums, double l1_scale, double ssim_scale, double constant, float* out, hipStream_t s);
void launch_l1_ssim_forward(int C, int H, int W, const float* img, const float* gt, float* Dmu, float* Ds1, float* Ds12,
                            double* sums, hipStream_t s);
void launch_l1_ssim_backward(int C, int H, int W, const float* img, const float* gt, const float* Dmu, const float* Ds1,
                             const float* Ds12, const float* grad_loss, float l1_coeff, float ssim_coeff, float* dL_dimg,
                             hipStream_t s);
constexpr int64_t IMAGE_METRICS_MAX_WORKGROUPS = (int64_t(1) << 24) - 1;
int64_t image_metrics_workgroups(int N, int C, int H, int W);
size_t image_metrics_ws_bytes(int N, int C, int H, int W);
void launch_image_metrics(int N, int C, int H, int W, const float* img, const float* gt, double* partials, double* out,
                          hipStream_t s);

size_t qat_workspace_bytes();
size_t qat_scan_bytes(int P);
void launch_qat_observe(const c3dgs_qat_params& q, void* workspace, hipStream_t s);
void launch_qat_codebooks(const c3dgs_qat_params& q, float* scales_n, float* rotations, float* shs, hipStream_t s);
void launch_qat_codebooks_backward(const c3dgs_qat_params& q, const float* g_scales, const float* g_rot, const float* g_shs,
                                   float* d_scaling, float* d_rotation, float* d_dc, float* d_rest, hipStream_t s);
hipError_t run_qat_visible(const c3dgs_qat_params& q, const float* view, uint8_t* visible, int32_t* rank, int32_t* count,
                           void* scan_ws, hipStream_t s);
void launch_qat_points(const c3dgs_qat_params& q, const uint8_t* visible, const int32_t* rank, const int64_t* sh_idx,
                       const int64_t* g_idx, float* means3D, float* opac, float* sfac, int64_t* sh_out, int64_t* g_out,
                       hipStream_t s);
void launch_qat_points_backward(const c3dgs_qat_params& q, const uint8_t* visible, const int32_t* rank, const float* g_m3,
                                const float* g_m2, const float* g_op, const float* g_sf, float* d_xyz, float* d_screen,
                                float* d_op, float* d_sf, hipStream_t s);
void launch_qat_quantize(const c3dgs_qat_params& q, int scaling_exp, int8_t* opacity, int8_t* scaling, int8_t* scaling_factor,
                         int8_t* rotation, int8_t* features_dc, int8_t* features_rest, hipStream_t s);
void launch_fake_quantize(long long n, const float* x, c3dgs_fq_state* state, int observe, int enabled, float c, float* out,
                          void* workspace, hipStream_t s);
void launch_fake_quantize_backward(long long n, const float* x, const c3dgs_fq_state* state, int enabled, const float* g,
                                   float* dx, hipStream_t s);

}
```

### c3dgs_amd/csrc/preprocess.hip

```cpp
#include "common.hpp"
#include "gsmath.hpp"

namespace c3dgs {

template <bool POSE>
__global__ void __launch_bounds__(256)
mark_visible_kernel(int P, const float* __restrict__ means3D, const float* __restrict__ view_or_pose, uint8_t* __restrict__ present, int vec)
{
    const int j = blockIdx.x * 256 + threadIdx.x;
    const int i0 = 4 * j;
    if (i0 >= P) return;
    float vm[16];
    const float* view = view_or_pose;
    if (POSE) {
        const float x = view_or_pose[0], y = view_or_pose[1], z = view_or_pose[2], w = view_or_pose[3], tz = view_or_pose[6];
        const float d2 = y * y + z * z + x * x;
#pragma unroll
        for (int q = 0; q < 16; q++) vm[q] = 0.f;
        vm[2] = 2.0f * (x * z - w * y); vm[6] = 2.0f * (y * z + w * x); vm[10] = 1.0f + 2.0f * (z * z - d2); vm[14] = tz;
        view = vm;
    }
    if (vec && i0 + 4 <= P) {
        const float4* src = reinterpret_cast<const float4*>(means3D) + 3 * (size_t)j;
        const float4 a = src[0], b = src[1], c = src[2];
        const f3 p0 = { a.x, a.y, a.z }, p1 = { a.w, b.x, b.y }, p2 = { b.z, b.w, c.x }, p3 = { c.y, c.z, c.w };
        const uint32_t v0 = !(xform4x3(p0, view).z <= 0.01f), v1 = !(xform4x3(p1, view).z <= 0.01f);
        const uint32_t v2 = !(xform4x3(p2, view).z <= 0.01f), v3 = !(xform4x3(p3, view).z <= 0.01f);
        reinterpret_cast<uint32_t*>(present)[j] = v0 | (v1 << 8) | (v2 << 16) | (v3 << 24);
        return;
    }
    for (int i = i0; i < min(i0 + 4, P); i++) {
        f3 p = { means3D[3 * (size_t)i], means3D[3 * (size_t)i + 1], means3D[3 * (size_t)i + 2] };
        f3 pv = xform4x3(p, view);
        present[i] = !(pv.z <= 0.01f) ? 1 : 0;
    }
}

__global__ void __launch_bounds__(256)
pack_codebook_kernel(int GS, const float* __restrict__ scales, const float* __restrict__ rotations, float4* __restrict__ gtab)
{
    const int g = blockIdx.x * 256 + threadIdx.x;
    if (g >= GS) return;
    gtab[2 * (size_t)g] = *reinterpret_cast<const float4*>(rotations + 4 * (size_t)g);
    gtab[2 * (size_t)g + 1] = make_float4(scales[3 * (size_t)g], scales[3 * (size_t)g + 1], scales[3 * (size_t)g + 2], 0.f);
}

void launch_pack_codebook(const c3dgs_raster_params& p, float4* gtab, hipStream_t s)
{
    if (p.GS <= 0) return;
    pack_codebook_kernel<<<(p.GS + 255) / 256, 256, 0, s>>>(p.GS, p.scales, p.rotations, gtab);
}

void launch_mark_visible(int P, const float* means3D, const float* view, uint8_t* present, hipStream_t s)
{
    if (P <= 0) return;
    const int vec = ((reinterpret_cast<uintptr_t>(means3D) & 15u) == 0 && (reinterpret_cast<uintptr_t>(present) & 3u) == 0) ? 1 : 0;
    mark_visible_kernel<false><<<((P + 3) / 4 + 255) / 256, 256, 0, s>>>(P, means3D, view, present, vec);
}

void launch_mark_visible_pose(int P, const float* means3D, const float* pose, uint8_t* present, hipStream_t s)
{
    if (P <= 0) return;
    const int vec = ((reinterpret_cast<uintptr_t>(means3D) & 15u) == 0 && (reinterpret_cast<uintptr_t>(present) & 3u) == 0) ? 1 : 0;
    mark_visible_kernel<true><<<((P + 3) / 4 + 255) / 256, 256, 0, s>>>(P, means3D, pose, present, vec);
}

__global__ void camera_from_pose_kernel(const float* __restrict__ pose, float inv_tan_x, float inv_tan_y, float pa, float pb,
                                        float* __restrict__ view, float* __restrict__ proj, float* __restrict__ campos)
{
    if (threadIdx.x != 0 || blockIdx.x != 0) return;
    const float x = pose[0], y = pose[1], z = pose[2], w = pose[3], tx = pose[4], ty = pose[5], tz = pose[6];
    const float d2 = y * y + z * z + x * x;
    float M[4][4];
    M[0][0] = 1.0f + 2.0f * (x * x - d2); M[0][1] = 2.0f * (x * y - w * z);        M[0][2] = 2.0f * (x * z + w * y);        M[0][3] = tx;
    M[1][0] = 2.0f * (x * y + w * z);        M[1][1] = 1.0f + 2.0f * (y * y - d2); M[1][2] = 2.0f * (y * z - w * x);        M[1][3] = ty;
    M[2][0] = 2.0f * (x * z - w * y);        M[2][1] = 2.0f * (y * z + w * x);        M[2][2] = 1.0f + 2.0f * (z * z - d2); M[2][3] = tz;
    M[3][0] = 0.f; M[3][1] = 0.f; M[3][2] = 0.f; M[3][3] = 1.f;
#pragma unroll
    for (int i = 0; i < 4; i++) {
#pragma unroll
        for (int j = 0; j < 4; j++) view[i * 4 + j] = M[j][i];
        proj[i * 4 + 0] = M[0][i] * inv_tan_x;
        proj[i * 4 + 1] = M[1][i] * inv_tan_y;
        proj[i * 4 + 2] = M[2][i] * pa + M[3][i] * pb;
        proj[i * 4 + 3] = M[2][i];
    }
    const double a = M[0][0], b = M[0][1], c = M[0][2], d = M[1][0], e = M[1][1], f = M[1][2], g = M[2][0], h = M[2][1], k = M[2][2];
    const double A = e * k - f * h, B = -(d * k - f * g), C = d * h - e * g;
    const double det = a * A + b * B + c * C;
    const double inv[3][3] = { { A / det, -(b * k - c * h) / det, (b * f - c * e) / det },
                               { B / det, (a * k - c * g) / det, -(a * f - c * d) / det },
                               { C / det, -(a * h - b * g) / det, (a * e - b * d) / det } };
#pragma unroll
    for (int r = 0; r < 3; r++) campos[r] = (float)-(inv[r][0] * (double)tx + inv[r][1] * (double)ty + inv[r][2] * (double)tz);
}

void launch_camera_from_pose(const float* pose, float inv_tan_x, float inv_tan_y, float* view, float* proj, float* campos, hipStream_t s)
{
    const float pa = (float)(1.0 * 100.0 / (100.0 - 0.01)), pb = (float)(-(100.0 * 0.01) / (100.0 - 0.01));
    camera_from_pose_kernel<<<1, 64, 0, s>>>(pose, inv_tan_x, inv_tan_y, pa, pb, view, proj, campos);
}

template <int DEG>
__device__ __forceinline__ void sh_to_rgb(const float* c, float x, float y, float z, float out[3])
{
#pragma unroll
    for (int ch = 0; ch < 3; ch++) {
        float res = SH_C0 * c[0 * 3 + ch];
        if (DEG > 0) {
            res = res - SH_C1 * y * c[1 * 3 + ch] + SH_C1 * z * c[2 * 3 + ch] - SH_C1 * x * c[3 * 3 + ch];
            if (DEG > 1) {
                float xx = x * x, yy = y * y, zz = z * z;
                float xy = x * y, yz = y * z, xz = x * z;
                res = res + SH_C2_0 * xy * c[4 * 3 + ch] + SH_C2_1 * yz * c[5 * 3 + ch] +
                      SH_C2_2 * (2.0f * zz - xx - yy) * c[6 * 3 + ch] + SH_C2_3 * xz * c[7 * 3 + ch] +
                      SH_C2_4 * (xx - yy) * c[8 * 3 + ch];
                if (DEG > 2) {
                    res = res + SH_C3_0 * y * (3.0f * xx - yy) * c[9 * 3 + ch] + SH_C3_1 * xy * z * c[10 * 3 + ch] +
                          SH_C3_2 * y * (4.0f * zz - xx - yy) * c[11 * 3 + ch] +
                          SH_C3_3 * z * (2.0f * zz - 3.0f * xx - 3.0f * yy) * c[12 * 3 + ch] +
                          SH_C3_4 * x * (4.0f * zz - xx - yy) * c[13 * 3 + ch] + SH_C3_5 * z * (xx - yy) * c[14 * 3 + ch] +
                          SH_C3_6 * x * (xx - 3.0f * yy) * c[15 * 3 + ch];
                }
            }
        }
        out[ch] = res + 0.5f;
    }
}

struct PreArgs {
    int P, M, W, H, gx, gy;
    const float* means3D; const float* sh; const float* colors_precomp; const float* opacities;
    const float* scales; const float* scale_factors; const float* rotations; const float* cov3D_precomp;
    const int64_t* sh_indices; const int64_t* g_indices;
    const float* view; const float* proj; const float* campos;
    float tan_fovx, tan_fovy, focal_x, focal_y, scale_modifier;
    int prefiltered, clamp_color;
    int32_t* radii; float4* splat; uint16_t* rects; uint8_t* clamped;
    uint32_t* depth_keys;
    uint32_t* inst_offset; uint32_t* block_total;
    uint2* ranges; int T;
    const float4* gtab;
    uint4* zero_span; size_t zero_n16;
};

template <int DEG>
__global__ void __launch_bounds__(256) preprocess_kernel(const PreArgs a)
{
    __shared__ uint32_t s_wsum[4];
    const int t = threadIdx.x, lane = t & 63, wave = t >> 6;
    const int i = blockIdx.x * 256 + t;
    const bool in_range = i < a.P;
    for (int q = i; q < a.T; q += gridDim.x * 256) a.ranges[q] = make_uint2(0u, 0u);
    if (a.zero_n16) {
        const size_t per = (a.zero_n16 + gridDim.x - 1) / gridDim.x, z0 = (size_t)blockIdx.x * per, z1 = min(z0 + per, a.zero_n16);
        for (size_t q = z0 + t; q < z1; q += 256) a.zero_span[q] = make_uint4(0u, 0u, 0u, 0u);
    }

    int32_t out_radius = 0;
    uint32_t out_tiles = 0;
    uint32_t out_key = 0xffffffffu;
    bool alive = false;
    float4 rec0 = make_float4(0, 0, 0, 0), rec1 = rec0;
    float rgb2 = 0.f;
    uint32_t rect_lo = 0, rect_hi = 0;
    if (in_range) do {
        const f3 p = { a.means3D[3 * (size_t)i], a.means3D[3 * (size_t)i + 1], a.means3D[3 * (size_t)i + 2] };
        const f3 p_view = xform4x3(p, a.view);
        if (!a.prefiltered && p_view.z <= 0.01f) break;

        const float4 p_hom = xform4x4(p, a.proj);
        const float p_w = 1.0f / (p_hom.w + 0.0000001f);
        const float projx = p_hom.x * p_w, projy = p_hom.y * p_w;

        float cov3D[6];
        if (a.cov3D_precomp) {
#pragma unroll
            for (int q = 0; q < 6; q++) cov3D[q] = a.cov3D_precomp[6 * (size_t)i + q];
        } else if (a.g_indices) {
            const size_t g = (size_t)a.g_indices[i];
            const float4 rot = a.gtab[2 * g], sc = a.gtab[2 * g + 1];
            cov3d_from_scale_rot(sc.x, sc.y, sc.z, a.scale_factors[i] * a.scale_modifier, rot, cov3D);
        } else {
            const float4 rot = *reinterpret_cast<const float4*>(a.rotations + 4 * (size_t)i);
            cov3d_from_scale_rot(a.scales[3 * (size_t)i], a.scales[3 * (size_t)i + 1], a.scales[3 * (size_t)i + 2],
                                 a.scale_modifier, rot, cov3D);
        }
        const Cov2D cv = cov2d(p, a.focal_x, a.focal_y, a.tan_fovx, a.tan_fovy, cov3D, a.view);

        const float det = (cv.a * cv.c - cv.b * cv.b);
        if (det == 0.0f) break;
        const float det_inv = 1.f / det;
        const float conic_a = cv.c * det_inv, conic_b = -cv.b * det_inv, conic_c = cv.a * det_inv;

        const float mid = 0.5f * (cv.a + cv.c);
        const float lambda1 = mid + sqrtf(fmaxf(0.1f, mid * mid - det));
        const float lambda2 = mid - sqrtf(fmaxf(0.1f, mid * mid - det));
        const float my_radius = ceilf(3.f * sqrtf(fmaxf(lambda1, lambda2)));
        const float pix = ndc2pix(projx, a.W), piy = ndc2pix(projy, a.H);
        int x0, y0, x1, y1;
        get_rect(pix, piy, (int)my_radius, a.gx, a.gy, x0, y0, x1, y1);
        if ((x1 - x0) * (y1 - y0) == 0) break;

        float rgb[3];
        uint8_t clamp_bits = 0;
        if (a.colors_precomp) {
            rgb[0] = a.colors_precomp[3 * (size_t)i];
            rgb[1] = a.colors_precomp[3 * (size_t)i + 1];
            rgb[2] = a.colors_precomp[3 * (size_t)i + 2];
        } else {
            const size_t row = a.sh_indices ? (size_t)a.sh_indices[i] : (size_t)i;
            const float* shp = a.sh + row * (size_t)a.M * 3;
            constexpr int NC = (DEG + 1) * (DEG + 1) * 3;
            float c[NC];
            if ((a.M * 3) % 4 == 0 && NC % 4 == 0) {
#pragma unroll
                for (int q = 0; q < NC / 4; q++) {
                    const float4 v = reinterpret_cast<const float4*>(shp)[q];
                    c[4 * q] = v.x; c[4 * q + 1] = v.y; c[4 * q + 2] = v.z; c[4 * q + 3] = v.w;
                }
            } else {
#pragma unroll
                for (int q = 0; q < NC; q++) c[q] = shp[q];
            }
            f3 dir = { p.x - a.campos[0], p.y - a.campos[1], p.z - a.campos[2] };
            const float len = sqrtf(dir.x * dir.x + dir.y * dir.y + dir.z * dir.z);
            dir.x = dir.x / len; dir.y = dir.y / len; dir.z = dir.z / len;
            sh_to_rgb<DEG>(c, dir.x, dir.y, dir.z, rgb);
            if (a.clamp_color) {
#pragma unroll
                for (int ch = 0; ch < 3; ch++) {
                    if (rgb[ch] < 0) clamp_bits |= (uint8_t)(1u << ch);
                    rgb[ch] = fmaxf(rgb[ch], 0.0f);
                }
            }
        }

        alive = true;
        out_radius = (int32_t)my_radius;
        out_tiles = (uint32_t)((y1 - y0) * (x1 - x0));
        out_key = __float_as_uint(p_view.z);
        a.clamped[i] = clamp_bits;
        uint16_t* rc = a.rects + 4 * (size_t)i;
        rc[0] = (uint16_t)x0; rc[1] = (uint16_t)y0; rc[2] = (uint16_t)x1; rc[3] = (uint16_t)y1;
        rec0 = make_float4(pix, piy, conic_a, conic_b);
        rec1 = make_float4(conic_c, a.opacities[i], rgb[0], rgb[1]);
        rgb2 = rgb[2];
        rect_lo = (uint32_t)x0 | ((uint32_t)y0 << 16);
        rect_hi = (uint32_t)x1 | ((uint32_t)y1 << 16);
    } while (false);

    uint32_t incl = out_tiles;
#pragma unroll
    for (int o = 1; o < 64; o <<= 1) { const uint32_t v = __shfl_up(incl, o); if (lane >= o) incl += v; }
    if (lane == 63) s_wsum[wave] = incl;
    __syncthreads();
    uint32_t woff = 0;
    for (int w = 0; w < wave; w++) woff += s_wsum[w];
    const uint32_t my_incl = woff + incl;
    if (t == 255) a.block_total[blockIdx.x] = my_incl;
    if (!in_range) return;
    if (!alive) *reinterpret_cast<uint2*>(a.rects + 4 * (size_t)i) = make_uint2(0u, 0u);
    if (alive) {
        float4* rec = a.splat + 3 * (size_t)i;
        rec[0] = rec0;
        rec[1] = rec1;
        rec[2] = make_float4(rgb2, __uint_as_float(my_incl - out_tiles), __uint_as_float(rect_lo), __uint_as_float(rect_hi));
    }
    a.inst_offset[i] = my_incl;
    a.radii[i] = out_radius;
    a.depth_keys[i] = out_key;
}

__global__ void __launch_bounds__(1024) scan_blocks_kernel(int nb, uint32_t* __restrict__ base, const uint32_t* __restrict__ sort_err,
                                                           uint32_t* __restrict__ host_out, uint32_t host_seq)
{
    __shared__ uint32_t s_w[2][16];
    const int t = threadIdx.x, lane = t & 63, wave = t >> 6;
    uint32_t carry = 0;
    int buf = 0;
    for (int c0 = 0; c0 < nb; c0 += 16384, buf ^= 1) {
        const int i0 = c0 + t * 16;
        uint32_t v[16];
#pragma unroll
        for (int q = 0; q < 4; q++) {
            uint4 x = make_uint4(0u, 0u, 0u, 0u);
            if (i0 + 4 * q + 3 < nb) x = reinterpret_cast<const uint4*>(base + i0)[q];
            else {
                if (i0 + 4 * q < nb) x.x = base[i0 + 4 * q];
                if (i0 + 4 * q + 1 < nb) x.y = base[i0 + 4 * q + 1];
                if (i0 + 4 * q + 2 < nb) x.z = base[i0 + 4 * q + 2];
            }
            v[4 * q] = x.x; v[4 * q + 1] = x.y; v[4 * q + 2] = x.z; v[4 * q + 3] = x.w;
        }
        uint32_t mine = 0;
#pragma unroll
        for (int q = 0; q < 16; q++) mine += v[q];
        uint32_t incl = mine;
#pragma unroll
        for (int o = 1; o < 64; o <<= 1) { const uint32_t u = __shfl_up(incl, o); if (lane >= o) incl += u; }
        if (lane == 63) s_w[buf][wave] = incl;
        __syncthreads();
        uint32_t off = carry, all = 0;
#pragma unroll
        for (int w = 0; w < 16; w++) { const uint32_t x = s_w[buf][w]; if (w < wave) off += x; all += x; }
        uint32_t run = off + incl - mine;
#pragma unroll
        for (int q = 0; q < 16; q++) { const uint32_t x = v[q]; v[q] = run; run += x; }
#pragma unroll
        for (int q = 0; q < 4; q++) {
            if (i0 + 4 * q + 3 < nb) reinterpret_cast<uint4*>(base + i0)[q] = make_uint4(v[4 * q], v[4 * q + 1], v[4 * q + 2], v[4 * q + 3]);
            else {
                if (i0 + 4 * q < nb) base[i0 + 4 * q] = v[4 * q];
                if (i0 + 4 * q + 1 < nb) base[i0 + 4 * q + 1] = v[4 * q + 1];
                if (i0 + 4 * q + 2 < nb) base[i0 + 4 * q + 2] = v[4 * q + 2];
            }
        }
        carry += all;
    }
    __syncthreads();
    if (t == 0) {
        base[nb] = carry;
        const uint32_t err = sort_err ? *sort_err : 0u;
        if (sort_err) base[nb + 1] = err;
        if (host_out) {
            __hip_atomic_store(host_out, carry, __ATOMIC_RELAXED, __HIP_MEMORY_SCOPE_SYSTEM);
            __hip_atomic_store(host_out + 1, err, __ATOMIC_RELAXED, __HIP_MEMORY_SCOPE_SYSTEM);
            __hip_atomic_store(host_out + 2, host_seq, __ATOMIC_RELEASE, __HIP_MEMORY_SCOPE_SYSTEM);
        }
    }
}

void launch_preprocess(const c3dgs_raster_params& p, const GeomPtrs& g, int32_t* radii, uint2* ranges, const uint32_t* sort_err,
                       void* zero_span, size_t zero_n16, uint32_t* host_out, uint32_t host_seq, hipStream_t s)
{
    if (p.P <= 0) return;
    PreArgs a;
    a.P = p.P; a.M = p.M; a.W = p.W; a.H = p.H; a.gx = tiles_x(p.W); a.gy = tiles_y(p.H);
    a.means3D = p.means3D; a.sh = p.sh; a.colors_precomp = p.colors_precomp; a.opacities = p.opacities;
    a.scales = p.scales; a.scale_factors = p.scale_factors; a.rotations = p.rotations; a.cov3D_precomp = p.cov3D_precomp;
    a.sh_indices = p.sh_indices; a.g_indices = p.g_indices;
    a.view = p.viewmatrix; a.proj = p.projmatrix; a.campos = p.campos;
    a.tan_fovx = p.tan_fovx; a.tan_fovy = p.tan_fovy;
    a.focal_y = p.H / (2.0f * p.tan_fovy);
    a.focal_x = p.W / (2.0f * p.tan_fovx);
    a.scale_modifier = p.scale_modifier; a.prefiltered = p.prefiltered; a.clamp_color = p.clamp_color;
    a.radii = radii; a.splat = g.splat; a.rects = g.rects;
    a.clamped = g.clamped; a.depth_keys = g.depth_keys;
    a.inst_offset = g.inst_offset;
    a.block_total = g.block_base;
    a.ranges = ranges; a.T = a.gx * a.gy;
    a.gtab = g.gtab;
    a.zero_span = (uint4*)zero_span; a.zero_n16 = zero_span ? zero_n16 : 0;
    const dim3 grid((p.P + 255) / 256), block(256);
    const int deg = p.colors_precomp ? 0 : p.D;
    switch (deg) {
        case 0: preprocess_kernel<0><<<grid, block, 0, s>>>(a); break;
        case 1: preprocess_kernel<1><<<grid, block, 0, s>>>(a); break;
        case 2: preprocess_kernel<2><<<grid, block, 0, s>>>(a); break;
        default: preprocess_kernel<3><<<grid, block, 0, s>>>(a); break;
    }
    scan_blocks_kernel<<<1, 1024, 0, s>>>((int)grid.x, g.block_base, sort_err, host_out, host_seq);
}

__device__ __forceinline__ uint32_t rect_tiles(const uint2 rc)
{
    return (uint32_t)(((int)(rc.y & 0xffff) - (int)(rc.x & 0xffff)) * ((int)(rc.y >> 16) - (int)(rc.x >> 16)));
}

__global__ void __launch_bounds__(256)
block_totals_kernel(int n, const uint2* __restrict__ rects_sorted, uint32_t* __restrict__ totals)
{
    __shared__ uint32_t s_w[4];
    const int i = blockIdx.x * 256 + threadIdx.x;
    uint32_t x = i < n ? rect_tiles(rects_sorted[i]) : 0u;
#pragma unroll
    for (int o = 32; o > 0; o >>= 1) x += __shfl_xor(x, o);
    if ((threadIdx.x & 63) == 0) s_w[threadIdx.x >> 6] = x;
    __syncthreads();
    if (threadIdx.x == 0) totals[blockIdx.x] = (s_w[0] + s_w[1]) + (s_w[2] + s_w[3]);
}

template <class K>
__global__ void __launch_bounds__(256)
duplicate_with_keys_kernel(int P, const uint32_t* __restrict__ order, const uint2* __restrict__ rects_sorted,
                           const uint32_t* __restrict__ depth_base, K* __restrict__ keys, uint32_t* __restrict__ values,
                           int grid_x, const uint32_t* __restrict__ sort_err, uint4* __restrict__ zero_span, size_t zero_n16)
{
    if (zero_n16) {
        const size_t per = (zero_n16 + gridDim.x - 1) / gridDim.x, z0 = (size_t)blockIdx.x * per, z1 = min(z0 + per, zero_n16);
        for (size_t q = z0 + threadIdx.x; q < z1; q += 256) zero_span[q] = make_uint4(0u, 0u, 0u, 0u);
    }
    if (*sort_err) return;
    __shared__ uint32_t s_end[256];
    __shared__ uint32_t s_id[256];
    __shared__ uint2 s_rect[256];
    __shared__ uint32_t s_inv[256];
    __shared__ uint32_t s_wsum[4];
    const int t = threadIdx.x, lane = t & 63, wave = t >> 6;
    const int k0 = blockIdx.x * 256, k = k0 + t;
    const uint32_t out_begin = depth_base[blockIdx.x];
    uint32_t incl = 0;
    if (k < P) {
        const uint2 rc = rects_sorted[k];
        incl = rect_tiles(rc);
        s_id[t] = order[k];
        s_rect[t] = rc;
        const uint32_t w = (rc.y & 0xffff) - (rc.x & 0xffff);
        s_inv[t] = w > 1 ? 0xffffffffu / w + 1u : 0u;
    }
#pragma unroll
    for (int o = 1; o < 64; o <<= 1) { const uint32_t v = __shfl_up(incl, o); if (lane >= o) incl += v; }
    if (lane == 63) s_wsum[wave] = incl;
    __syncthreads();
    uint32_t woff = out_begin;
    for (int w = 0; w < wave; w++) woff += s_wsum[w];
    s_end[t] = woff + incl;
    __syncthreads();
    const int nk = min(256, P - k0);
    const uint32_t out_end = s_end[nk - 1];
    constexpr int CH = 1024;
    __shared__ uint16_t s_head[CH];
    __shared__ uint32_t s_wmax[4];
    const uint32_t my_tiles = k < P ? rect_tiles(s_rect[t]) : 0u;
    const uint32_t my_begin = s_end[t] - my_tiles;
    uint32_t carry = 0;
    for (uint32_t c0 = out_begin & ~3u; c0 < out_end; c0 += CH) {
        reinterpret_cast<uint2*>(s_head)[t] = make_uint2(0u, 0u);
        __syncthreads();
        if (my_tiles && my_begin >= c0 && my_begin < c0 + CH) s_head[my_begin - c0] = (uint16_t)(t + 1);
        __syncthreads();
        const uint2 hv = reinterpret_cast<const uint2*>(s_head)[t];
        uint32_t m[4] = { hv.x & 0xffffu, hv.x >> 16, hv.y & 0xffffu, hv.y >> 16 };
        m[1] = max(m[0], m[1]); m[2] = max(m[1], m[2]); m[3] = max(m[2], m[3]);
        uint32_t scan = m[3];
#pragma unroll
        for (int o = 1; o < 64; o <<= 1) { const uint32_t v = __shfl_up(scan, o); if (lane >= o) scan = max(scan, v); }
        uint32_t before = __shfl_up(scan, 1);
        if (lane == 0) before = 0;
        if (lane == 63) s_wmax[wave] = scan;
        __syncthreads();
        before = max(before, carry);
        for (int w = 0; w < wave; w++) before = max(before, s_wmax[w]);
        carry = max(max(carry, max(s_wmax[0], s_wmax[1])), max(s_wmax[2], s_wmax[3]));
        const uint32_t o0 = c0 + 4u * t;
        K kq[4];
        uint32_t vq[4];
#pragma unroll
        for (int e = 0; e < 4; e++) {
            const uint32_t o = o0 + e;
            const uint32_t own = max(before, m[e]);
            kq[e] = 0; vq[e] = 0;
            if (o >= out_begin && o < out_end) {
                const int g = (int)own - 1;
                const uint32_t first = (g == 0) ? out_begin : s_end[g - 1];
                const uint2 rc = s_rect[g];
                const int x0 = rc.x & 0xffff, y0 = rc.x >> 16, x1 = rc.y & 0xffff;
                const uint32_t local = o - first, w = (uint32_t)(x1 - x0), inv = s_inv[g];
                const uint32_t ry = inv ? __umulhi(local, inv) : local, rx = local - ry * w;
                kq[e] = (K)((y0 + ry) * grid_x + (x0 + rx));
                vq[e] = s_id[g];
            }
        }
        if (o0 >= out_begin && o0 + 4 <= out_end) {
            if constexpr (sizeof(K) == 2)
                *reinterpret_cast<uint2*>(keys + o0) = make_uint2((uint32_t)kq[0] | ((uint32_t)kq[1] << 16), (uint32_t)kq[2] | ((uint32_t)kq[3] << 16));
            else
                *reinterpret_cast<uint4*>(keys + o0) = make_uint4((uint32_t)kq[0], (uint32_t)kq[1], (uint32_t)kq[2], (uint32_t)kq[3]);
            *reinterpret_cast<uint4*>(values + o0) = make_uint4(vq[0], vq[1], vq[2], vq[3]);
        } else {
#pragma unroll
            for (int e = 0; e < 4; e++)
                if (o0 + e >= out_begin && o0 + e < out_end) { keys[o0 + e] = kq[e]; values[o0 + e] = vq[e]; }
        }
        __syncthreads();
    }
}

void launch_depth_order_scan(int P, const GeomPtrs& g, hipStream_t s)
{
    if (P <= 0) return;
    const int nb = (P + 255) / 256;
    block_totals_kernel<<<nb, 256, 0, s>>>(P, g.sorted_offsets, g.depth_base);
    scan_blocks_kernel<<<1, 1024, 0, s>>>(nb, g.depth_base, nullptr, nullptr, 0u);
}

void launch_duplicate_with_keys(int P, const GeomPtrs& g, const BinPtrs& b, int grid_x, const uint32_t* sort_err,
                                void* zero_span, size_t zero_n16, hipStream_t s)
{
    if (P <= 0) return;
    if (!zero_span) zero_n16 = 0;
    if (b.key_bytes == 4)
        duplicate_with_keys_kernel<uint32_t><<<(P + 255) / 256, 256, 0, s>>>(P, g.depth_order, g.sorted_offsets, g.depth_base,
                                                                             (uint32_t*)b.keys_unsorted, b.values_unsorted, grid_x, sort_err, (uint4*)zero_span, zero_n16);
    else
        duplicate_with_keys_kernel<uint16_t><<<(P + 255) / 256, 256, 0, s>>>(P, g.depth_order, g.sorted_offsets, g.depth_base,
                                                                             (uint16_t*)b.keys_unsorted, b.values_unsorted, grid_x, sort_err, (uint4*)zero_span, zero_n16);
}

template <class K>
__global__ void __launch_bounds__(256)
identify_ranges_kernel(int L, const K* __restrict__ keys, uint2* __restrict__ ranges, const uint32_t* __restrict__ sort_err)
{
    if (*sort_err) return;
    const int j = blockIdx.x * 256 + threadIdx.x;
    const int i0 = j * 8;
    if (i0 >= L) return;
    uint32_t cur8[8];
    if constexpr (sizeof(K) == 2) {
        const uint4 v = reinterpret_cast<const uint4*>(keys)[j];
        const uint32_t w[4] = { v.x, v.y, v.z, v.w };
#pragma unroll
        for (int e = 0; e < 8; e++) cur8[e] = (e & 1) ? (w[e >> 1] >> 16) : (w[e >> 1] & 0xffffu);
    } else {
        const uint4 v0 = reinterpret_cast<const uint4*>(keys)[2 * j], v1 = reinterpret_cast<const uint4*>(keys)[2 * j + 1];
        cur8[0] = v0.x; cur8[1] = v0.y; cur8[2] = v0.z; cur8[3] = v0.w; cur8[4] = v1.x; cur8[5] = v1.y; cur8[6] = v1.z; cur8[7] = v1.w;
    }
    uint32_t prev = i0 > 0 ? (uint32_t)keys[i0 - 1] : 0xffffffffu;
#pragma unroll
    for (int e = 0; e < 8; e++) {
        const int idx = i0 + e;
        if (idx < L) {
            const uint32_t cur = cur8[e];
            if (cur != prev) {
                if (idx > 0) ranges[prev].y = (uint32_t)idx;
                ranges[cur].x = (uint32_t)idx;
            }
            if (idx == L - 1) ranges[cur].y = (uint32_t)L;
            prev = cur;
        }
    }
}

void launch_identify_ranges(int R, const void* keys_sorted, int key_bytes, uint2* ranges, const uint32_t* sort_err, hipStream_t s)
{
    if (R <= 0) return;
    const int threads = (R + 7) / 8;
    if (key_bytes == 4) identify_ranges_kernel<uint32_t><<<(threads + 255) / 256, 256, 0, s>>>(R, (const uint32_t*)keys_sorted, ranges, sort_err);
    else identify_ranges_kernel<uint16_t><<<(threads + 255) / 256, 256, 0, s>>>(R, (const uint16_t*)keys_sorted, ranges, sort_err);
}

}
```

### c3dgs_amd/csrc/radix_sort.hip

```cpp
#include "common.hpp"
#include <algorithm>
#include <cstdlib>

namespace c3dgs {

constexpr int OS_RADIX = 256;
#ifndef C3DGS_OS_TILE32
#define C3DGS_OS_TILE32 12288
#endif
#ifndef C3DGS_OS_BLOCK32
#define C3DGS_OS_BLOCK32 512
#endif
constexpr int OS_TILE16 = 8192, OS_BLOCK16 = 1024;
template <class K> struct OsShape {
    static constexpr int TILE = sizeof(K) == 2 ? OS_TILE16 : C3DGS_OS_TILE32;
    static constexpr int BLOCK = sizeof(K) == 2 ? OS_BLOCK16 : C3DGS_OS_BLOCK32;
    static constexpr int IPT = TILE / BLOCK;
};
constexpr uint32_t OS_FLAG_AGG = 1u << 30, OS_FLAG_PRE = 2u << 30, OS_CNT_MASK = (1u << 30) - 1;
constexpr int OS_MAX_PASSES = 4;
#ifndef C3DGS_OS_SPIN_LIMIT
#define C3DGS_OS_SPIN_LIMIT (1u << 22)
#endif
constexpr uint32_t OS_SPIN_LIMIT = C3DGS_OS_SPIN_LIMIT;
__device__ uint32_t g_os_error;
#ifdef C3DGS_DIAG
__device__ unsigned long long g_os_times[64 * 8];
#endif
#ifdef C3DGS_OS_TIMING
#define OS_T(slot) if (tid == 0 && (bid & 3) == 0 && (bid >> 2) < 64) g_os_times[(bid >> 2) * 8 + (slot)] = __builtin_readcyclecounter();
#define OS_T_DRAIN() asm volatile("s_waitcnt vmcnt(0)");
#define OS_T_LOADS_DONE()                                                                                    \
    if (key[0] == (K)0x12345678 && val[OS_IPT - 1] == 0x87654321u) kout[0] = key[OS_IPT - 1];                \
    OS_T_DRAIN()
#else
#define OS_T(slot)
#define OS_T_DRAIN()
#define OS_T_LOADS_DONE()
#endif

struct OsPlan { int passes; int bits[OS_MAX_PASSES]; };

static OsPlan os_plan(int total_bits)
{
    OsPlan p;
    p.passes = (total_bits + 7) / 8;
    if (p.passes < 1) p.passes = 1;
    int left = total_bits < 1 ? 1 : total_bits;
    for (int i = 0; i < p.passes; i++) {
        const int b = (left + (p.passes - i) - 1) / (p.passes - i);
        p.bits[i] = b;
        left -= b;
    }
    return p;
}

template <class K> static size_t os_blocks(size_t n) { return (n + OsShape<K>::TILE - 1) / OsShape<K>::TILE; }
template <class K> constexpr bool os_pre_pass0() { return sizeof(K) == 2; }
constexpr int OS_TABLE_ROW = 2 * OS_RADIX;
template <class K> static size_t os_table_words(size_t n) { return os_pre_pass0<K>() ? os_blocks<K>(n) * OS_TABLE_ROW : 0; }
template <class K> static size_t os_ctrl_bytes(size_t n, int passes)
{
    return align_up(((size_t)passes * OS_RADIX + (size_t)passes * os_blocks<K>(n) * OS_RADIX + 64 + os_table_words<K>(n)) * sizeof(uint32_t));
}

constexpr int OS_HIST_BLOCK = 1024;
template <class K>
__global__ void __launch_bounds__(OS_HIST_BLOCK) os_hist_kernel(const K* __restrict__ keys, size_t n, OsPlan plan, uint32_t* __restrict__ hist)
{
    __shared__ uint32_t s_h[OS_MAX_PASSES][OS_RADIX];
    for (int q = threadIdx.x; q < OS_MAX_PASSES * OS_RADIX; q += OS_HIST_BLOCK) (&s_h[0][0])[q] = 0;
    __syncthreads();
    constexpr int VEC = 16 / sizeof(K);
    const size_t nvec = n / VEC;
    const uint4* k4 = reinterpret_cast<const uint4*>(keys);
    auto add = [&](uint32_t k) {
        int shift = 0;
        for (int p = 0; p < plan.passes; p++) {
            atomicAdd(&s_h[p][(k >> shift) & ((1u << plan.bits[p]) - 1u)], 1u);
            shift += plan.bits[p];
        }
    };
    auto add4 = [&](const uint4 v) {
        const uint32_t w[4] = { v.x, v.y, v.z, v.w };
#pragma unroll
        for (int e = 0; e < 4; e++) {
            if (sizeof(K) == 4) add(w[e]);
            else { add(w[e] & 0xffffu); add(w[e] >> 16); }
        }
    };
    const size_t stride = (size_t)gridDim.x * OS_HIST_BLOCK;
    size_t i = (size_t)blockIdx.x * OS_HIST_BLOCK + threadIdx.x;
    for (; i + 3 * stride < nvec; i += 4 * stride) {
        const uint4 v0 = k4[i], v1 = k4[i + stride], v2 = k4[i + 2 * stride], v3 = k4[i + 3 * stride];
        add4(v0); add4(v1); add4(v2); add4(v3);
    }
    for (; i < nvec; i += stride) add4(k4[i]);
    for (size_t j = nvec * VEC + (size_t)blockIdx.x * OS_HIST_BLOCK + threadIdx.x; j < n; j += stride) add((uint32_t)keys[j]);
    __syncthreads();
    for (int q = threadIdx.x; q < plan.passes * OS_RADIX; q += OS_HIST_BLOCK) {
        const uint32_t v = (&s_h[0][0])[q];
        if (v) atomicAdd(&hist[q], v);
    }
}

__global__ void __launch_bounds__(1024) os_tile_hist_kernel(const uint16_t* __restrict__ keys, uint32_t n, OsPlan plan, uint32_t* __restrict__ table)
{
    constexpr int TILE = OsShape<uint16_t>::TILE;
    static_assert(TILE == 8 * 1024, "one 16-byte load of 8 keys per thread");
    __shared__ uint32_t s_h[OS_TABLE_ROW];
    if (threadIdx.x < OS_TABLE_ROW) s_h[threadIdx.x] = 0;
    __syncthreads();
    const uint32_t base = blockIdx.x * (uint32_t)TILE + threadIdx.x * 8u;
    const uint32_t m0 = (1u << plan.bits[0]) - 1u, m1 = plan.passes > 1 ? (1u << plan.bits[1]) - 1u : 0u;
    auto add = [&](uint32_t k) {
        atomicAdd(&s_h[k & m0], 1u);
        if (plan.passes > 1) atomicAdd(&s_h[OS_RADIX + ((k >> plan.bits[0]) & m1)], 1u);
    };
    if (base + 8 <= n && (reinterpret_cast<uintptr_t>(keys) & 15u) == 0) {
        const uint4 v = *reinterpret_cast<const uint4*>(keys + base);
        const uint32_t w[4] = { v.x, v.y, v.z, v.w };
#pragma unroll
        for (int e = 0; e < 4; e++) { add(w[e] & 0xffffu); add(w[e] >> 16); }
    } else {
        for (uint32_t i = base; i < min(base + 8u, n); i++) add((uint32_t)keys[i]);
    }
    __syncthreads();
    const int t = threadIdx.x;
    if (t < OS_TABLE_ROW && (t >> 8) < plan.passes && (t & (OS_RADIX - 1)) < (1 << plan.bits[(t >> 8) & 1]))
        table[(size_t)t * gridDim.x + blockIdx.x] = s_h[t];
}

__global__ void __launch_bounds__(256) os_table_scan_kernel(uint32_t* __restrict__ table, uint32_t blocks, OsPlan plan, uint32_t* __restrict__ hist)
{
    __shared__ uint32_t s_w[4];
    const int n0 = 1 << plan.bits[0];
    const int pass = (int)blockIdx.x < n0 ? 0 : 1, digit = (int)blockIdx.x - (pass ? n0 : 0), col = pass * OS_RADIX + digit;
    uint32_t* column = table + (size_t)col * blocks;
    const int lane = threadIdx.x & 63, wave = threadIdx.x >> 6;
    uint32_t carry = 0;
    for (uint32_t b0 = 0; b0 < blocks; b0 += 256) {
        const uint32_t b = b0 + threadIdx.x;
        const uint32_t c = b < blocks ? column[b] : 0u;
        uint32_t incl = c;
#pragma unroll
        for (int o = 1; o < 64; o <<= 1) { const uint32_t t = __shfl_up(incl, o); if (lane >= o) incl += t; }
        __syncthreads();
        if (lane == 63) s_w[wave] = incl;
        __syncthreads();
        uint32_t off = carry;
        for (int w = 0; w < wave; w++) off += s_w[w];
        if (pass == 0 && b < blocks) column[b] = off + incl - c;
        carry += s_w[0] + s_w[1] + s_w[2] + s_w[3];
    }
    if (threadIdx.x == 0) hist[col] = carry;
}

__device__ __forceinline__ uint32_t os_load(const uint32_t* p) { return __hip_atomic_load(p, __ATOMIC_RELAXED, __HIP_MEMORY_SCOPE_AGENT); }
__device__ __forceinline__ void os_store(uint32_t* p, uint32_t v) { __hip_atomic_store(p, v, __ATOMIC_RELAXED, __HIP_MEMORY_SCOPE_AGENT); }

__device__ __forceinline__ uint32_t os_pack_rect(uint2 r)
{
    return (r.x & 0xffu) | ((r.x >> 16) << 8) | ((r.y & 0xffu) << 16) | ((r.y >> 16) << 24);
}
__device__ __forceinline__ uint2 os_unpack_rect(uint32_t w)
{
    return make_uint2((w & 0xffu) | (((w >> 8) & 0xffu) << 16), ((w >> 16) & 0xffu) | ((w >> 24) << 16));
}

template <class K, int BITS, bool PRE, bool PAY2 = false>
__global__ void __launch_bounds__(OsShape<K>::BLOCK)
os_pass_kernel(const K* __restrict__ kin, K* __restrict__ kout, const uint32_t* __restrict__ vin, uint32_t* __restrict__ vout,
               uint32_t n, int shift, const uint32_t* __restrict__ hist, uint32_t* __restrict__ status, uint32_t* __restrict__ ticket,
               const uint2* __restrict__ gather_src, uint2* __restrict__ gather_dst, const uint32_t* __restrict__ p2in = nullptr,
               uint32_t* __restrict__ p2out = nullptr)
{
    constexpr uint32_t ERR_BIT = sizeof(K) == 2 ? 1u : 2u;
    constexpr uint32_t MASK = (1u << BITS) - 1;
    constexpr int OS_BLOCK = OsShape<K>::BLOCK, OS_IPT = OsShape<K>::IPT, OS_WAVES = OS_BLOCK / 64;
    __shared__ uint32_t s_cnt[OS_WAVES][OS_RADIX];
    __shared__ uint32_t s_start[OS_RADIX];
    __shared__ int32_t s_gbase[OS_RADIX];
    __shared__ uint32_t s_wtot[4];
    __shared__ uint32_t s_bid;
    constexpr int OS_TILE = OsShape<K>::TILE;
    __shared__ K s_keys[OS_TILE];
    __shared__ uint32_t s_vals[OS_TILE];
    __shared__ uint32_t s_vals2[PAY2 ? OS_TILE : 1];

    const int tid = threadIdx.x, lane = tid & 63, wave = tid >> 6;
    if (tid == 0) s_bid = PRE ? blockIdx.x : atomicAdd(ticket, 1u);
    for (int q = tid; q < OS_WAVES * OS_RADIX; q += OS_BLOCK) (&s_cnt[0][0])[q] = 0;
    __syncthreads();
    const uint32_t bid = s_bid;
    OS_T(0)
    const uint32_t block_start = bid * (uint32_t)OS_TILE;
    const uint32_t valid = min((uint32_t)OS_TILE, n - block_start);

    K key[OS_IPT];
    uint32_t val[OS_IPT], rank[OS_IPT];
    uint32_t val2[PAY2 ? OS_IPT : 1];
    const uint32_t wbase = block_start + (uint32_t)wave * 64u * OS_IPT;
#pragma unroll
    for (int k = 0; k < OS_IPT; k++) {
        const uint32_t idx = wbase + (uint32_t)k * 64u + lane;
        const bool ok = idx < n;
        key[k] = ok ? kin[idx] : (K)0;
        val[k] = ok ? (vin ? vin[idx] : idx) : 0u;
        if (PAY2) val2[k] = ok ? (p2in ? p2in[idx] : os_pack_rect(gather_src[idx])) : 0u;
    }
    const uint32_t lt_lo = lane < 32 ? (1u << lane) - 1u : 0xffffffffu, lt_hi = lane < 32 ? 0u : (1u << (lane - 32)) - 1u;
    OS_T_LOADS_DONE()
    OS_T(1)
    uint32_t* wc = s_cnt[wave];
#pragma unroll
    for (int k = 0; k < OS_IPT; k++) {
        const uint32_t idx = wbase + (uint32_t)k * 64u + lane;
        const bool ok = idx < n;
        const uint32_t d = ((uint32_t)key[k] >> shift) & MASK;
        const unsigned long long okb = __ballot(ok);
        uint32_t plo = (uint32_t)okb, phi = (uint32_t)(okb >> 32);
#pragma unroll
        for (int b = 0; b < BITS; b++) {
            const int sgn = __builtin_amdgcn_sbfe((int)d, b, 1);
            const unsigned long long bal = __ballot(sgn != 0);
            plo &= ~((uint32_t)bal ^ (uint32_t)sgn);
            phi &= ~((uint32_t)(bal >> 32) ^ (uint32_t)sgn);
        }
        rank[k] = 0;
        if (ok) {
            const uint32_t before = __hip_atomic_load(&wc[d], __ATOMIC_RELAXED, __HIP_MEMORY_SCOPE_WAVEFRONT);
            const uint32_t below = (uint32_t)__popc(plo & lt_lo) + (uint32_t)__popc(phi & lt_hi);
            rank[k] = before + below;
            if (below == 0) __hip_atomic_store(&wc[d], before + (uint32_t)__popc(plo) + (uint32_t)__popc(phi), __ATOMIC_RELAXED, __HIP_MEMORY_SCOPE_WAVEFRONT);
        }
        __builtin_amdgcn_fence(__ATOMIC_RELEASE, "wavefront");
        __builtin_amdgcn_wave_barrier();
        __builtin_amdgcn_fence(__ATOMIC_ACQUIRE, "wavefront");
    }
    OS_T(2)
    __syncthreads();
    OS_T(3)
    uint32_t tot = 0;
    if (tid < OS_RADIX) {
#pragma unroll
        for (int w = 0; w < OS_WAVES; w++) { const uint32_t c = s_cnt[w][tid]; s_cnt[w][tid] = tot; tot += c; }
    }
    uint32_t incl = tot;
#pragma unroll
    for (int o = 1; o < 64; o <<= 1) { const uint32_t t = __shfl_up(incl, o); if (lane >= o) incl += t; }
    if (tid < OS_RADIX && lane == 63) s_wtot[wave] = incl;
    __syncthreads();
    uint32_t start = 0, pre = 0;
    if (tid < OS_RADIX) {
        uint32_t off = 0;
        for (int w = 0; w < wave; w++) off += s_wtot[w];
        start = off + incl - tot;
        s_start[tid] = start;
        uint32_t* my = status + (size_t)bid * OS_RADIX + tid;
        if (PRE) pre = tid < (1 << BITS) ? status[(size_t)tid * gridDim.x + bid] : 0u;
        else if (bid == 0) os_store(my, OS_FLAG_PRE | tot);
        else {
            os_store(my, OS_FLAG_AGG | tot);
            for (int64_t b = (int64_t)bid - 1;; b--) {
                uint32_t s, spins = 0;
                do { s = os_load(status + (size_t)b * OS_RADIX + tid); } while ((s >> 30) == 0 && ++spins < OS_SPIN_LIMIT);
                if ((s >> 30) == 0) { atomicOr(&g_os_error, ERR_BIT); break; }
                pre += s & OS_CNT_MASK;
                if (s & OS_FLAG_PRE) break;
            }
            os_store(my, OS_FLAG_PRE | (pre + tot));
        }
    }
    OS_T(4)
    const uint32_t h = tid < OS_RADIX ? hist[tid] : 0u;
    uint32_t hincl = h;
#pragma unroll
    for (int o = 1; o < 64; o <<= 1) { const uint32_t t = __shfl_up(hincl, o); if (lane >= o) hincl += t; }
    __syncthreads();
    if (tid < OS_RADIX && lane == 63) s_wtot[wave] = hincl;
    __syncthreads();
    if (tid < OS_RADIX) {
        uint32_t off = 0;
        for (int w = 0; w < wave; w++) off += s_wtot[w];
        s_gbase[tid] = (int32_t)(off + hincl - h + pre) - (int32_t)start;
    }
    OS_T(5)
#pragma unroll
    for (int k = 0; k < OS_IPT; k++) {
        const uint32_t idx = wbase + (uint32_t)k * 64u + lane;
        if (idx < n) {
            const uint32_t d = ((uint32_t)key[k] >> shift) & MASK;
            const uint32_t p = s_start[d] + s_cnt[wave][d] + rank[k];
            s_keys[p] = key[k];
            s_vals[p] = val[k];
            if (PAY2) s_vals2[p] = val2[k];
        }
    }
    __syncthreads();
    OS_T(6)
#pragma unroll
    for (int m = 0; m < OS_IPT; m++) {
        const uint32_t p = (uint32_t)tid + (uint32_t)m * OS_BLOCK;
        if (p < valid) {
            const K kk = s_keys[p];
            const uint32_t d = ((uint32_t)kk >> shift) & MASK;
            const uint32_t g = (uint32_t)(s_gbase[d] + (int32_t)p);
            kout[g] = kk;
            const uint32_t vv = s_vals[p];
            vout[g] = vv;
            if (PAY2) {
                if (p2out) p2out[g] = s_vals2[p];
                else gather_dst[g] = os_unpack_rect(s_vals2[p]);
            } else if (gather_src) gather_dst[g] = gather_src[vv];
        }
    }
    OS_T_DRAIN()
    OS_T(7)
}

template <class K, bool PRE>
static void os_launch_pass(int bits, unsigned blocks, hipStream_t s, const K* ki, K* ko, const uint32_t* vi, uint32_t* vo, uint32_t n,
                           int shift, const uint32_t* hist, uint32_t* status, uint32_t* ticket, const uint2* gsrc, uint2* gdst)
{
#define C3DGS_OS_CASE(B) case B: os_pass_kernel<K, B, PRE><<<blocks, OsShape<K>::BLOCK, 0, s>>>(ki, ko, vi, vo, n, shift, hist, status, ticket, gsrc, gdst); break
    switch (bits) {
        C3DGS_OS_CASE(1); C3DGS_OS_CASE(2); C3DGS_OS_CASE(3); C3DGS_OS_CASE(4);
        C3DGS_OS_CASE(5); C3DGS_OS_CASE(6); C3DGS_OS_CASE(7);
        default: os_pass_kernel<K, 8, PRE><<<blocks, OsShape<K>::BLOCK, 0, s>>>(ki, ko, vi, vo, n, shift, hist, status, ticket, gsrc, gdst); break;
    }
#undef C3DGS_OS_CASE
}

template <class K>
static size_t os_temp_bytes(size_t n, int total_bits, bool pay2 = false)
{
    const OsPlan plan = os_plan(total_bits);
    size_t b = os_ctrl_bytes<K>(n, plan.passes);
    const int bufs = plan.passes >= 3 ? 2 : (plan.passes == 2 ? 1 : 0);
    b += (size_t)bufs * (align_up(n * sizeof(K)) + align_up(n * sizeof(uint32_t)));
    if (pay2) b += 2 * align_up(n * sizeof(uint32_t));
    return b;
}

template <class K>
static size_t os_clear_bytes(size_t n, int total_bits)
{
    const OsPlan plan = os_plan(total_bits);
    if (!os_pre_pass0<K>()) return os_ctrl_bytes<K>(n, plan.passes);
    return ((size_t)plan.passes * OS_RADIX + (size_t)plan.passes * os_blocks<K>(n) * OS_RADIX + 64) * sizeof(uint32_t);
}

template <class K>
static hipError_t os_sort(void* temp, size_t temp_bytes, const K* kin, K* kout, const uint32_t* vin, uint32_t* vout, size_t n,
                          int total_bits, hipStream_t s, const uint2* gather_src = nullptr, uint2* gather_dst = nullptr,
                          bool ctrl_cleared = false, bool pay2 = false)
{
    if (n == 0) return hipSuccess;
    if (pay2 && (sizeof(K) != 4 || total_bits != 32 || !gather_src || !gather_dst || vin || os_temp_bytes<K>(n, total_bits, true) > temp_bytes))
        pay2 = false;
    if (n >= ((size_t)1 << 30) || os_temp_bytes<K>(n, total_bits) > temp_bytes) return hipErrorInvalidValue;
    const OsPlan plan = os_plan(total_bits);
    if (os_pre_pass0<K>() && plan.passes > 2) return hipErrorInvalidValue;
    const size_t blocks = os_blocks<K>(n);
    char* base = (char*)temp;
    const size_t ctrl = os_ctrl_bytes<K>(n, plan.passes);
    uint32_t* hist = (uint32_t*)base;
    uint32_t* status = hist + (size_t)plan.passes * OS_RADIX;
    uint32_t* ticket = status + (size_t)plan.passes * blocks * OS_RADIX;
    uint32_t* table = ticket + 64;
    constexpr bool pre0 = os_pre_pass0<K>();
    K* tk[2]; uint32_t* tv[2];
    char* q = base + ctrl;
    for (int i = 0; i < 2; i++) { tk[i] = (K*)q; q += align_up(n * sizeof(K)); tv[i] = (uint32_t*)q; q += align_up(n * sizeof(uint32_t)); }
    uint32_t* t2[2] = { nullptr, nullptr };
    if (pay2) {
        q = base + os_temp_bytes<K>(n, total_bits);
        for (int i = 0; i < 2; i++) { t2[i] = (uint32_t*)q; q += align_up(n * sizeof(uint32_t)); }
    }
    if (!ctrl_cleared) {
        const hipError_t e = hipMemsetAsync(base, 0, os_clear_bytes<K>(n, total_bits), s);
        if (e != hipSuccess) return e;
    }
    if constexpr (pre0) {
        os_tile_hist_kernel<<<(unsigned)blocks, 1024, 0, s>>>((const uint16_t*)kin, (uint32_t)n, plan, table);
        os_table_scan_kernel<<<(unsigned)((1 << plan.bits[0]) + (plan.passes > 1 ? (1 << plan.bits[1]) : 0)), 256, 0, s>>>(table, (uint32_t)blocks, plan, hist);
    } else {
        const size_t nvec16 = n * sizeof(K) / 16 + 1;
        const unsigned hb = (unsigned)std::min<size_t>((nvec16 + OS_HIST_BLOCK * 4 - 1) / (OS_HIST_BLOCK * 4), 512);
        os_hist_kernel<K><<<hb, OS_HIST_BLOCK, 0, s>>>(kin, n, plan, hist);
    }
    int shift = 0;
    for (int p = 0; p < plan.passes; p++) {
        const K* ki = p == 0 ? kin : tk[(p - 1) & 1];
        const uint32_t* vi = p == 0 ? vin : tv[(p - 1) & 1];
        K* ko = p == plan.passes - 1 ? kout : tk[p & 1];
        uint32_t* vo = p == plan.passes - 1 ? vout : tv[p & 1];
        const bool last = p == plan.passes - 1;
        if constexpr (sizeof(K) == 4) {
            if (pay2) {
                os_pass_kernel<K, 8, false, true><<<(unsigned)blocks, OsShape<K>::BLOCK, 0, s>>>(
                    ki, ko, vi, vo, (uint32_t)n, shift, hist + (size_t)p * OS_RADIX, status + (size_t)p * blocks * OS_RADIX, ticket + p,
                    gather_src, gather_dst, p == 0 ? nullptr : t2[(p - 1) & 1], last ? nullptr : t2[p & 1]);
                shift += plan.bits[p];
                continue;
            }
        }
        if (pre0 && p == 0)
            os_launch_pass<K, true>(plan.bits[p], (unsigned)blocks, s, ki, ko, vi, vo, (uint32_t)n, shift, hist, table, ticket,
                                    last ? gather_src : nullptr, last ? gather_dst : nullptr);
        else
            os_launch_pass<K, false>(plan.bits[p], (unsigned)blocks, s, ki, ko, vi, vo, (uint32_t)n, shift, hist + (size_t)p * OS_RADIX,
                                     status + (size_t)p * blocks * OS_RADIX, ticket + p, last ? gather_src : nullptr, last ? gather_dst : nullptr);
        shift += plan.bits[p];
    }
    return hipGetLastError();
}

#ifdef C3DGS_DIAG
int os_read_times(unsigned long long* out512)
{
    return hipMemcpyFromSymbol(out512, HIP_SYMBOL(g_os_times), sizeof(unsigned long long) * 512) != hipSuccess;
}
#endif

uint32_t* onesweep_error_word()
{
    static uint32_t* cache[64] = { nullptr };
    int dev = 0;
    if (hipGetDevice(&dev) != hipSuccess || dev < 0 || dev >= 64) return nullptr;
    if (!cache[dev]) {
        void* p = nullptr;
        if (hipGetSymbolAddress(&p, HIP_SYMBOL(g_os_error)) != hipSuccess) return nullptr;
        cache[dev] = (uint32_t*)p;
    }
    return cache[dev];
}

int onesweep_timed_out(hipStream_t s)
{
    if (!onesweep_enabled()) return 0;
    uint32_t* e = onesweep_error_word();
    uint32_t w = 1;
    if (!e || hipMemcpyAsync(&w, e, sizeof(w), hipMemcpyDeviceToHost, s) != hipSuccess) return 1;
    if (hipStreamSynchronize(s) != hipSuccess) return 1;
    if (w) (void)hipMemsetAsync(e, 0, sizeof(w), s);
    return w != 0;
}

bool onesweep_enabled()
{
    static const bool on = []() { const char* e = std::getenv("C3DGS_SORT_ROCPRIM"); return !(e && e[0] == '1'); }();
    return on;
}
size_t onesweep_depth_temp_bytes(int P) { return os_temp_bytes<uint32_t>((size_t)(P > 0 ? P : 1), 32, true); }
size_t onesweep_tile_temp_bytes(int R, int end_bit, int key_bytes)
{
    return key_bytes == 4 ? os_temp_bytes<uint32_t>((size_t)(R > 0 ? R : 1), end_bit) : os_temp_bytes<uint16_t>((size_t)(R > 0 ? R : 1), end_bit);
}
size_t onesweep_depth_clear_bytes(int P) { return os_clear_bytes<uint32_t>((size_t)(P > 0 ? P : 1), 32); }
size_t onesweep_tile_clear_bytes(int R, int end_bit, int key_bytes)
{
    return key_bytes == 4 ? os_clear_bytes<uint32_t>((size_t)(R > 0 ? R : 1), end_bit) : os_clear_bytes<uint16_t>((size_t)(R > 0 ? R : 1), end_bit);
}
hipError_t onesweep_tile_sort32(void* temp, size_t temp_bytes, const uint32_t* kin, uint32_t* kout, const uint32_t* vin, uint32_t* vout,
                                int R, int end_bit, hipStream_t s, bool ctrl_cleared)
{
    return os_sort<uint32_t>(temp, temp_bytes, kin, kout, vin, vout, (size_t)R, end_bit, s, nullptr, nullptr, ctrl_cleared);
}
hipError_t onesweep_depth_sort(void* temp, size_t temp_bytes, const uint32_t* kin, uint32_t* kout, const uint32_t* vin, uint32_t* vout,
                               int P, const uint2* gather_src, uint2* gather_dst, hipStream_t s, bool ctrl_cleared, bool rects_fit_bytes)
{
    static const bool no_pay2 = []() { const char* e = std::getenv("C3DGS_DEPTH_SORT_GATHER"); return e && e[0] == '1'; }();
    return os_sort<uint32_t>(temp, temp_bytes, kin, kout, vin, vout, (size_t)P, 32, s, gather_src, gather_dst, ctrl_cleared,
                             rects_fit_bytes && !no_pay2);
}
hipError_t onesweep_tile_sort(void* temp, size_t temp_bytes, const uint16_t* kin, uint16_t* kout, const uint32_t* vin, uint32_t* vout,
                              int R, int end_bit, hipStream_t s, bool ctrl_cleared)
{
    return os_sort<uint16_t>(temp, temp_bytes, kin, kout, vin, vout, (size_t)R, end_bit, s, nullptr, nullptr, ctrl_cleared);
}

}
```

Baseline: 623.0 views/s.

## Fuse block-scan into depth-sort histogram kernel and restructure tile sort table passes

The single-workgroup block-offset scan after preprocess now runs as block 0 of the depth-sort histogram kernel, with the remaining blocks computing the onesweep histogram. The depth sort then skips its own histogram launch. This removes one kernel launch and lets the serial one-block scan overlap with histogram work. The 16-bit tile sort path is also restructured into a per-pass table-driven scheme with a per-pass hist and table-scan kernel, which changes the control-buffer layout.

```diff
diff --git a/c3dgs_amd/build.py b/c3dgs_amd/build.py
--- a/c3dgs_amd/build.py
+++ b/c3dgs_amd/build.py
@@ -35,7 +35,7 @@
     "image_io.hip": ["-ffp-contract=off"],
 }
 HEADERS = [os.path.join(CSRC, "common.hpp"), os.path.join(CSRC, "gsmath.hpp"), os.path.join(CSRC, "render_diag.hpp"),
-           os.path.join(CSRC, "render_common.hpp"),
+           os.path.join(CSRC, "render_common.hpp"), os.path.join(CSRC, "scan_blocks.hpp"),
            os.path.join(HERE, "..", "include", "c3dgs_hip.h"), os.path.join(HERE, "..", "include", "c3dgs_hip_debug.h")]
 
 
diff --git a/c3dgs_amd/csrc/binning.hip b/c3dgs_amd/csrc/binning.hip
--- a/c3dgs_amd/csrc/binning.hip
+++ b/c3dgs_amd/csrc/binning.hip
@@ -47,12 +47,19 @@
     return (onesweep_enabled() && (size_t)R < ((size_t)1 << 30)) ? onesweep_tile_clear_bytes(R, end_bit, key_bytes) : 0;
 }
 
+hipError_t run_depth_hist_scan(void* temp, size_t temp_bytes, const uint32_t* keys, int P, int nb, uint32_t* base,
+                               const uint32_t* sort_err, uint32_t* host_out, uint32_t host_seq, hipStream_t s)
+{
+    if (depth_sort_clear_bytes(P) == 0) return hipErrorInvalidValue;
+    return onesweep_depth_hist_scan(temp, temp_bytes, keys, P, nb, base, sort_err, host_out, host_seq, s);
+}
+
 hipError_t run_depth_sort(void* temp, size_t temp_bytes, const uint32_t* kin, uint32_t* kout, const uint32_t* vin,
                           uint32_t* vout, int P, const uint2* rects, uint2* rects_sorted, hipStream_t s, bool ctrl_cleared,
-                          bool rects_fit_bytes)
+                          bool rects_fit_bytes, bool hist_done)
 {
     if (onesweep_enabled() && (size_t)P < ((size_t)1 << 30))
-        return onesweep_depth_sort(temp, temp_bytes, kin, kout, vin, vout, P, rects, rects_sorted, s, ctrl_cleared, rects_fit_bytes);
+        return onesweep_depth_sort(temp, temp_bytes, kin, kout, vin, vout, P, rects, rects_sorted, s, ctrl_cleared, rects_fit_bytes, hist_done);
     hipError_t e = vin ? rocprim::radix_sort_pairs(temp, temp_bytes, kin, kout, vin, vout, (size_t)P, 0u, 32u, s)
                        : rocprim::radix_sort_pairs(temp, temp_bytes, kin, kout, rocprim::counting_iterator<uint32_t>(0u), vout,
                                                    (size_t)P, 0u, 32u, s);
diff --git a/c3dgs_amd/csrc/c_abi.hip b/c3dgs_amd/csrc/c_abi.hip
--- a/c3dgs_amd/csrc/c_abi.hip
+++ b/c3dgs_amd/csrc/c_abi.hip
@@ -203,16 +203,22 @@
     if (!hr.pinned) return fail(C3DGS_E_HIP, "pinned host buffer allocation failed");
     const uint32_t host_seq = hr.begin();
     const size_t dclear = depth_sort_clear_bytes(P) <= g.scan_temp_bytes ? depth_sort_clear_bytes(P) : 0;
+    const bool hist_with_scan = dclear != 0;
+    const int nb = (P + 255) / 256;
     { StageTimer t_(ST_PREPROCESS, s);
       if (geom_gtab_bytes(p)) launch_pack_codebook(p, g.gtab, s);
-      launch_preprocess(p, g, radii, img.ranges, sort_err, g.scan_temp, dclear / 16, hr.dev, host_seq, s); }
+      launch_preprocess(p, g, radii, img.ranges, g.scan_temp, dclear / 16, s);
+      if (hist_with_scan)
+          C3DGS_HIP_TRY(run_depth_hist_scan(g.scan_temp, g.scan_temp_bytes, g.depth_keys, P, nb, g.block_base, sort_err, hr.dev, host_seq, s));
+      else
+          launch_scan_blocks(nb, g.block_base, sort_err, hr.dev, host_seq, s); }
     C3DGS_STAGE_CHECK(ST_PREPROCESS, p.debug, s);
-    const uint32_t* r_words = g.block_base + (P + 255) / 256;
+    const uint32_t* r_words = g.block_base + nb;
     if (int rc = hr.queue_copy(r_words, s)) return rc;
     { StageTimer t_(ST_DEPTH_SORT, s);
       C3DGS_HIP_TRY(run_depth_sort(g.scan_temp, g.scan_temp_bytes, g.depth_keys, g.depth_keys_sorted, nullptr, g.depth_order, P,
                                    reinterpret_cast<const uint2*>(g.rects), g.sorted_offsets, s, dclear != 0,
-                                   gx <= 255 && gy <= 255)); }
+                                   gx <= 255 && gy <= 255, hist_with_scan)); }
     C3DGS_STAGE_CHECK(ST_DEPTH_SORT, p.debug, s);
     if (p.debug && onesweep_timed_out(s)) return fail(C3DGS_E_HIP, "depth sort: look-back timed out");
     C3DGS_TIMED_STAGE(ST_SCAN, p.debug, s, launch_depth_order_scan(P, g, s));
diff --git a/c3dgs_amd/csrc/common.hpp b/c3dgs_amd/csrc/common.hpp
--- a/c3dgs_amd/csrc/common.hpp
+++ b/c3dgs_amd/csrc/common.hpp
@@ -200,15 +200,18 @@
 void launch_mark_visible(int P, const float* means3D, const float* view, uint8_t* present, hipStream_t s);
 void launch_mark_visible_pose(int P, const float* means3D, const float* pose7, uint8_t* present, hipStream_t s);
 void launch_pack_codebook(const c3dgs_raster_params& p, float4* gtab, hipStream_t s);
-void launch_preprocess(const c3dgs_raster_params& p, const GeomPtrs& g, int32_t* radii, uint2* ranges, const uint32_t* sort_err,
-                       void* zero_span, size_t zero_n16, uint32_t* host_out, uint32_t host_seq, hipStream_t s);
+void launch_preprocess(const c3dgs_raster_params& p, const GeomPtrs& g, int32_t* radii, uint2* ranges, void* zero_span, size_t zero_n16,
+                       hipStream_t s);
+void launch_scan_blocks(int nb, uint32_t* base, const uint32_t* sort_err, uint32_t* host_out, uint32_t host_seq, hipStream_t s);
 void launch_depth_order_scan(int P, const GeomPtrs& g, hipStream_t s);
 void launch_duplicate_with_keys(int P, const GeomPtrs& g, const BinPtrs& b, int grid_x, const uint32_t* sort_err,
                                 void* zero_span, size_t zero_n16, hipStream_t s);
 void launch_identify_ranges(int R, const void* keys_sorted, int key_bytes, uint2* ranges, const uint32_t* sort_err, hipStream_t s);
 hipError_t run_depth_sort(void* temp, size_t temp_bytes, const uint32_t* kin, uint32_t* kout, const uint32_t* vin,
                           uint32_t* vout, int P, const uint2* rects, uint2* rects_sorted, hipStream_t s, bool ctrl_cleared = false,
-                          bool rects_fit_bytes = false);
+                          bool rects_fit_bytes = false, bool hist_done = false);
+hipError_t run_depth_hist_scan(void* temp, size_t temp_bytes, const uint32_t* keys, int P, int nb, uint32_t* base,
+                               const uint32_t* sort_err, uint32_t* host_out, uint32_t host_seq, hipStream_t s);
 hipError_t run_tile_sort(void* temp, size_t temp_bytes, const void* kin, void* kout, int key_bytes, const uint32_t* vin,
                          uint32_t* vout, int R, int end_bit, hipStream_t s, bool ctrl_cleared = false);
 size_t depth_sort_clear_bytes(int P);
@@ -222,7 +225,9 @@
 size_t onesweep_tile_clear_bytes(int R, int end_bit, int key_bytes);
 hipError_t onesweep_depth_sort(void* temp, size_t temp_bytes, const uint32_t* kin, uint32_t* kout, const uint32_t* vin, uint32_t* vout,
                                int P, const uint2* gather_src, uint2* gather_dst, hipStream_t s, bool ctrl_cleared = false,
-                               bool rects_fit_bytes = false);
+                               bool rects_fit_bytes = false, bool hist_done = false);
+hipError_t onesweep_depth_hist_scan(void* temp, size_t temp_bytes, const uint32_t* keys, int P, int nb, uint32_t* base,
+                                    const uint32_t* sort_err, uint32_t* host_out, uint32_t host_seq, hipStream_t s);
 hipError_t onesweep_tile_sort32(void* temp, size_t temp_bytes, const uint32_t* kin, uint32_t* kout, const uint32_t* vin, uint32_t* vout,
                                 int R, int end_bit, hipStream_t s, bool ctrl_cleared = false);
 hipError_t onesweep_tile_sort(void* temp, size_t temp_bytes, const uint16_t* kin, uint16_t* kout, const uint32_t* vin, uint32_t* vout,
diff --git a/c3dgs_amd/csrc/preprocess.hip b/c3dgs_amd/csrc/preprocess.hip
--- a/c3dgs_amd/csrc/preprocess.hip
+++ b/c3dgs_amd/csrc/preprocess.hip
@@ -1,5 +1,6 @@
 #include "common.hpp"
 #include "gsmath.hpp"
+#include "scan_blocks.hpp"
 
 namespace c3dgs {
 
@@ -272,67 +273,19 @@
     a.depth_keys[i] = out_key;
 }
 
-__global__ void __launch_bounds__(1024) scan_blocks_kernel(int nb, uint32_t* __restrict__ base, const uint32_t* __restrict__ sort_err,
-                                                           uint32_t* __restrict__ host_out, uint32_t host_seq)
-{
-    __shared__ uint32_t s_w[2][16];
-    const int t = threadIdx.x, lane = t & 63, wave = t >> 6;
-    uint32_t carry = 0;
-    int buf = 0;
-    for (int c0 = 0; c0 < nb; c0 += 16384, buf ^= 1) {
-        const int i0 = c0 + t * 16;
-        uint32_t v[16];
-#pragma unroll
-        for (int q = 0; q < 4; q++) {
-            uint4 x = make_uint4(0u, 0u, 0u, 0u);
-            if (i0 + 4 * q + 3 < nb) x = reinterpret_cast<const uint4*>(base + i0)[q];
-            else {
-                if (i0 + 4 * q < nb) x.x = base[i0 + 4 * q];
-                if (i0 + 4 * q + 1 < nb) x.y = base[i0 + 4 * q + 1];
-                if (i0 + 4 * q + 2 < nb) x.z = base[i0 + 4 * q + 2];
-            }
-            v[4 * q] = x.x; v[4 * q + 1] = x.y; v[4 * q + 2] = x.z; v[4 * q + 3] = x.w;
-        }
-        uint32_t mine = 0;
-#pragma unroll
-        for (int q = 0; q < 16; q++) mine += v[q];
-        uint32_t incl = mine;
-#pragma unroll
-        for (int o = 1; o < 64; o <<= 1) { const uint32_t u = __shfl_up(incl, o); if (lane >= o) incl += u; }
-        if (lane == 63) s_w[buf][wave] = incl;
-        __syncthreads();
-        uint32_t off = carry, all = 0;
-#pragma unroll
-        for (int w = 0; w < 16; w++) { const uint32_t x = s_w[buf][w]; if (w < wave) off += x; all += x; }
-        uint32_t run = off + incl - mine;
-#pragma unroll
-        for (int q = 0; q < 16; q++) { const uint32_t x = v[q]; v[q] = run; run += x; }
-#pragma unroll
-        for (int q = 0; q < 4; q++) {
-            if (i0 + 4 * q + 3 < nb) reinterpret_cast<uint4*>(base + i0)[q] = make_uint4(v[4 * q], v[4 * q + 1], v[4 * q + 2], v[4 * q + 3]);
-            else {
-                if (i0 + 4 * q < nb) base[i0 + 4 * q] = v[4 * q];
-                if (i0 + 4 * q + 1 < nb) base[i0 + 4 * q + 1] = v[4 * q + 1];
-                if (i0 + 4 * q + 2 < nb) base[i0 + 4 * q + 2] = v[4 * q + 2];
-            }
-        }
-        carry += all;
-    }
-    __syncthreads();
-    if (t == 0) {
-        base[nb] = carry;
-        const uint32_t err = sort_err ? *sort_err : 0u;
-        if (sort_err) base[nb + 1] = err;
-        if (host_out) {
-            __hip_atomic_store(host_out, carry, __ATOMIC_RELAXED, __HIP_MEMORY_SCOPE_SYSTEM);
-            __hip_atomic_store(host_out + 1, err, __ATOMIC_RELAXED, __HIP_MEMORY_SCOPE_SYSTEM);
-            __hip_atomic_store(host_out + 2, host_seq, __ATOMIC_RELEASE, __HIP_MEMORY_SCOPE_SYSTEM);
-        }
-    }
-}
-
-void launch_preprocess(const c3dgs_raster_params& p, const GeomPtrs& g, int32_t* radii, uint2* ranges, const uint32_t* sort_err,
-                       void* zero_span, size_t zero_n16, uint32_t* host_out, uint32_t host_seq, hipStream_t s)
+__global__ void __launch_bounds__(SCAN_BLOCKS_THREADS) scan_blocks_kernel(int nb, uint32_t* __restrict__ base, const uint32_t* __restrict__ sort_err,
+                                                                          uint32_t* __restrict__ host_out, uint32_t host_seq)
+{
+    scan_blocks_body(nb, base, sort_err, host_out, host_seq);
+}
+
+void launch_scan_blocks(int nb, uint32_t* base, const uint32_t* sort_err, uint32_t* host_out, uint32_t host_seq, hipStream_t s)
+{
+    scan_blocks_kernel<<<1, SCAN_BLOCKS_THREADS, 0, s>>>(nb, base, sort_err, host_out, host_seq);
+}
+
+void launch_preprocess(const c3dgs_raster_params& p, const GeomPtrs& g, int32_t* radii, uint2* ranges, void* zero_span, size_t zero_n16,
+                       hipStream_t s)
 {
     if (p.P <= 0) return;
     PreArgs a;
@@ -360,7 +313,6 @@
         case 2: preprocess_kernel<2><<<grid, block, 0, s>>>(a); break;
         default: preprocess_kernel<3><<<grid, block, 0, s>>>(a); break;
     }
-    scan_blocks_kernel<<<1, 1024, 0, s>>>((int)grid.x, g.block_base, sort_err, host_out, host_seq);
 }
 
 __device__ __forceinline__ uint32_t rect_tiles(const uint2 rc)
@@ -482,7 +434,7 @@
     if (P <= 0) return;
     const int nb = (P + 255) / 256;
     block_totals_kernel<<<nb, 256, 0, s>>>(P, g.sorted_offsets, g.depth_base);
-    scan_blocks_kernel<<<1, 1024, 0, s>>>(nb, g.depth_base, nullptr, nullptr, 0u);
+    launch_scan_blocks(nb, g.depth_base, nullptr, nullptr, 0u, s);
 }
 
 void launch_duplicate_with_keys(int P, const GeomPtrs& g, const BinPtrs& b, int grid_x, const uint32_t* sort_err,
diff --git a/c3dgs_amd/csrc/radix_sort.hip b/c3dgs_amd/csrc/radix_sort.hip
--- a/c3dgs_amd/csrc/radix_sort.hip
+++ b/c3dgs_amd/csrc/radix_sort.hip
@@ -1,4 +1,5 @@
 #include "common.hpp"
+#include "scan_blocks.hpp"
 #include <algorithm>
 #include <cstdlib>
 
@@ -56,17 +57,21 @@
 }
 
 template <class K> static size_t os_blocks(size_t n) { return (n + OsShape<K>::TILE - 1) / OsShape<K>::TILE; }
-template <class K> constexpr bool os_pre_pass0() { return sizeof(K) == 2; }
-constexpr int OS_TABLE_ROW = 2 * OS_RADIX;
-template <class K> static size_t os_table_words(size_t n) { return os_pre_pass0<K>() ? os_blocks<K>(n) * OS_TABLE_ROW : 0; }
+template <class K> constexpr bool os_table_driven() { return sizeof(K) == 2; }
+template <class K> static size_t os_table_words(size_t n) { return os_table_driven<K>() ? os_blocks<K>(n) * OS_RADIX : 0; }
+template <class K> static size_t os_lookback_words(size_t n, int passes)
+{
+    return os_table_driven<K>() ? 0 : (size_t)passes * os_blocks<K>(n) * OS_RADIX + 64;
+}
 template <class K> static size_t os_ctrl_bytes(size_t n, int passes)
 {
-    return align_up(((size_t)passes * OS_RADIX + (size_t)passes * os_blocks<K>(n) * OS_RADIX + 64 + os_table_words<K>(n)) * sizeof(uint32_t));
+    return align_up(((size_t)passes * OS_RADIX + os_lookback_words<K>(n, passes) + os_table_words<K>(n)) * sizeof(uint32_t));
 }
 
 constexpr int OS_HIST_BLOCK = 1024;
 template <class K>
-__global__ void __launch_bounds__(OS_HIST_BLOCK) os_hist_kernel(const K* __restrict__ keys, size_t n, OsPlan plan, uint32_t* __restrict__ hist)
+__device__ __forceinline__ void os_hist_body(const K* __restrict__ keys, size_t n, const OsPlan& plan, uint32_t* __restrict__ hist,
+                                             unsigned block, unsigned nblocks)
 {
     __shared__ uint32_t s_h[OS_MAX_PASSES][OS_RADIX];
     for (int q = threadIdx.x; q < OS_MAX_PASSES * OS_RADIX; q += OS_HIST_BLOCK) (&s_h[0][0])[q] = 0;
@@ -89,14 +94,14 @@
             else { add(w[e] & 0xffffu); add(w[e] >> 16); }
         }
     };
-    const size_t stride = (size_t)gridDim.x * OS_HIST_BLOCK;
-    size_t i = (size_t)blockIdx.x * OS_HIST_BLOCK + threadIdx.x;
+    const size_t stride = (size_t)nblocks * OS_HIST_BLOCK;
+    size_t i = (size_t)block * OS_HIST_BLOCK + threadIdx.x;
     for (; i + 3 * stride < nvec; i += 4 * stride) {
         const uint4 v0 = k4[i], v1 = k4[i + stride], v2 = k4[i + 2 * stride], v3 = k4[i + 3 * stride];
         add4(v0); add4(v1); add4(v2); add4(v3);
     }
     for (; i < nvec; i += stride) add4(k4[i]);
-    for (size_t j = nvec * VEC + (size_t)blockIdx.x * OS_HIST_BLOCK + threadIdx.x; j < n; j += stride) add((uint32_t)keys[j]);
+    for (size_t j = nvec * VEC + (size_t)block * OS_HIST_BLOCK + threadIdx.x; j < n; j += stride) add((uint32_t)keys[j]);
     __syncthreads();
     for (int q = threadIdx.x; q < plan.passes * OS_RADIX; q += OS_HIST_BLOCK) {
         const uint32_t v = (&s_h[0][0])[q];
@@ -104,19 +109,31 @@
     }
 }
 
-__global__ void __launch_bounds__(1024) os_tile_hist_kernel(const uint16_t* __restrict__ keys, uint32_t n, OsPlan plan, uint32_t* __restrict__ table)
+template <class K>
+__global__ void __launch_bounds__(OS_HIST_BLOCK) os_hist_kernel(const K* __restrict__ keys, size_t n, OsPlan plan, uint32_t* __restrict__ hist)
+{
+    os_hist_body<K>(keys, n, plan, hist, blockIdx.x, gridDim.x);
+}
+
+static_assert(SCAN_BLOCKS_THREADS == OS_HIST_BLOCK, "one workgroup shape for both bodies");
+__global__ void __launch_bounds__(OS_HIST_BLOCK)
+os_hist_scan_kernel(const uint32_t* __restrict__ keys, size_t n, OsPlan plan, uint32_t* __restrict__ hist, int nb, uint32_t* __restrict__ base,
+                    const uint32_t* __restrict__ sort_err, uint32_t* __restrict__ host_out, uint32_t host_seq)
+{
+    if (blockIdx.x == 0) scan_blocks_body(nb, base, sort_err, host_out, host_seq);
+    else os_hist_body<uint32_t>(keys, n, plan, hist, blockIdx.x - 1, gridDim.x - 1);
+}
+
+__global__ void __launch_bounds__(1024) os_tile_hist_kernel(const uint16_t* __restrict__ keys, uint32_t n, int shift, int bits, uint32_t* __restrict__ table)
 {
     constexpr int TILE = OsShape<uint16_t>::TILE;
     static_assert(TILE == 8 * 1024, "one 16-byte load of 8 keys per thread");
-    __shared__ uint32_t s_h[OS_TABLE_ROW];
-    if (threadIdx.x < OS_TABLE_ROW) s_h[threadIdx.x] = 0;
+    __shared__ uint32_t s_h[OS_RADIX];
+    if (threadIdx.x < OS_RADIX) s_h[threadIdx.x] = 0;
     __syncthreads();
     const uint32_t base = blockIdx.x * (uint32_t)TILE + threadIdx.x * 8u;
-    const uint32_t m0 = (1u << plan.bits[0]) - 1u, m1 = plan.passes > 1 ? (1u << plan.bits[1]) - 1u : 0u;
-    auto add = [&](uint32_t k) {
-        atomicAdd(&s_h[k & m0], 1u);
-        if (plan.passes > 1) atomicAdd(&s_h[OS_RADIX + ((k >> plan.bits[0]) & m1)], 1u);
-    };
+    const uint32_t mask = (1u << bits) - 1u;
+    auto add = [&](uint32_t k) { atomicAdd(&s_h[(k >> shift) & mask], 1u); };
     if (base + 8 <= n && (reinterpret_cast<uintptr_t>(keys) & 15u) == 0) {
         const uint4 v = *reinterpret_cast<const uint4*>(keys + base);
         const uint32_t w[4] = { v.x, v.y, v.z, v.w };
@@ -127,33 +144,37 @@
     }
     __syncthreads();
     const int t = threadIdx.x;
-    if (t < OS_TABLE_ROW && (t >> 8) < plan.passes && (t & (OS_RADIX - 1)) < (1 << plan.bits[(t >> 8) & 1]))
-        table[(size_t)t * gridDim.x + blockIdx.x] = s_h[t];
-}
-
-__global__ void __launch_bounds__(256) os_table_scan_kernel(uint32_t* __restrict__ table, uint32_t blocks, OsPlan plan, uint32_t* __restrict__ hist)
-{
+    if (t < (1 << bits)) table[(size_t)t * gridDim.x + blockIdx.x] = s_h[t];
+}
+
+constexpr int OS_SCAN_V = 8;
+__global__ void __launch_bounds__(256) os_table_scan_kernel(uint32_t* __restrict__ table, uint32_t blocks, uint32_t* __restrict__ hist)
+{
+    static_assert(OS_RADIX == 256, "one thread per histogram word");
     __shared__ uint32_t s_w[4];
-    const int n0 = 1 << plan.bits[0];
-    const int pass = (int)blockIdx.x < n0 ? 0 : 1, digit = (int)blockIdx.x - (pass ? n0 : 0), col = pass * OS_RADIX + digit;
-    uint32_t* column = table + (size_t)col * blocks;
+    const int digit = (int)blockIdx.x;
+    uint32_t* column = table + (size_t)digit * blocks;
     const int lane = threadIdx.x & 63, wave = threadIdx.x >> 6;
+    if (digit == 0 && threadIdx.x >= gridDim.x) hist[threadIdx.x] = 0u;
     uint32_t carry = 0;
-    for (uint32_t b0 = 0; b0 < blocks; b0 += 256) {
-        const uint32_t b = b0 + threadIdx.x;
-        const uint32_t c = b < blocks ? column[b] : 0u;
-        uint32_t incl = c;
+    for (uint32_t b0 = 0; b0 < blocks; b0 += 256 * OS_SCAN_V) {
+        const uint32_t b = b0 + threadIdx.x * OS_SCAN_V;
+        uint32_t c[OS_SCAN_V], mine = 0;
+#pragma unroll
+        for (int q = 0; q < OS_SCAN_V; q++) { c[q] = b + q < blocks ? column[b + q] : 0u; mine += c[q]; }
+        uint32_t incl = mine;
 #pragma unroll
         for (int o = 1; o < 64; o <<= 1) { const uint32_t t = __shfl_up(incl, o); if (lane >= o) incl += t; }
         __syncthreads();
         if (lane == 63) s_w[wave] = incl;
         __syncthreads();
-        uint32_t off = carry;
-        for (int w = 0; w < wave; w++) off += s_w[w];
-        if (pass == 0 && b < blocks) column[b] = off + incl - c;
+        uint32_t run = carry + incl - mine;
+        for (int w = 0; w < wave; w++) run += s_w[w];
+#pragma unroll
+        for (int q = 0; q < OS_SCAN_V; q++) { if (b + q < blocks) column[b + q] = run; run += c[q]; }
         carry += s_w[0] + s_w[1] + s_w[2] + s_w[3];
     }
-    if (threadIdx.x == 0) hist[col] = carry;
+    if (threadIdx.x == 0) hist[digit] = carry;
 }
 
 __device__ __forceinline__ uint32_t os_load(const uint32_t* p) { return __hip_atomic_load(p, __ATOMIC_RELAXED, __HIP_MEMORY_SCOPE_AGENT); }
@@ -332,6 +353,12 @@
 #undef C3DGS_OS_CASE
 }
 
+template <class K> static unsigned os_hist_blocks(size_t n)
+{
+    const size_t nvec16 = n * sizeof(K) / 16 + 1;
+    return (unsigned)std::min<size_t>((nvec16 + OS_HIST_BLOCK * 4 - 1) / (OS_HIST_BLOCK * 4), 512);
+}
+
 template <class K>
 static size_t os_temp_bytes(size_t n, int total_bits, bool pay2 = false)
 {
@@ -346,75 +373,74 @@
 template <class K>
 static size_t os_clear_bytes(size_t n, int total_bits)
 {
-    const OsPlan plan = os_plan(total_bits);
-    if (!os_pre_pass0<K>()) return os_ctrl_bytes<K>(n, plan.passes);
-    return ((size_t)plan.passes * OS_RADIX + (size_t)plan.passes * os_blocks<K>(n) * OS_RADIX + 64) * sizeof(uint32_t);
+    if (os_table_driven<K>()) return 0;
+    return os_ctrl_bytes<K>(n, os_plan(total_bits).passes);
 }
 
 template <class K>
 static hipError_t os_sort(void* temp, size_t temp_bytes, const K* kin, K* kout, const uint32_t* vin, uint32_t* vout, size_t n,
                           int total_bits, hipStream_t s, const uint2* gather_src = nullptr, uint2* gather_dst = nullptr,
-                          bool ctrl_cleared = false, bool pay2 = false)
+                          bool ctrl_cleared = false, bool pay2 = false, bool hist_done = false)
 {
     if (n == 0) return hipSuccess;
     if (pay2 && (sizeof(K) != 4 || total_bits != 32 || !gather_src || !gather_dst || vin || os_temp_bytes<K>(n, total_bits, true) > temp_bytes))
         pay2 = false;
-    if (n >= ((size_t)1 << 30) || os_temp_bytes<K>(n, total_bits) > temp_bytes) return hipErrorInvalidValue;
+    if (n >= ((size_t)1 << 30) || total_bits > 8 * (int)sizeof(K) || os_temp_bytes<K>(n, total_bits) > temp_bytes) return hipErrorInvalidValue;
     const OsPlan plan = os_plan(total_bits);
-    if (os_pre_pass0<K>() && plan.passes > 2) return hipErrorInvalidValue;
     const size_t blocks = os_blocks<K>(n);
     char* base = (char*)temp;
     const size_t ctrl = os_ctrl_bytes<K>(n, plan.passes);
     uint32_t* hist = (uint32_t*)base;
-    uint32_t* status = hist + (size_t)plan.passes * OS_RADIX;
-    uint32_t* ticket = status + (size_t)plan.passes * blocks * OS_RADIX;
-    uint32_t* table = ticket + 64;
-    constexpr bool pre0 = os_pre_pass0<K>();
+    uint32_t* behind_hist = hist + (size_t)plan.passes * OS_RADIX;
     K* tk[2]; uint32_t* tv[2];
     char* q = base + ctrl;
     for (int i = 0; i < 2; i++) { tk[i] = (K*)q; q += align_up(n * sizeof(K)); tv[i] = (uint32_t*)q; q += align_up(n * sizeof(uint32_t)); }
-    uint32_t* t2[2] = { nullptr, nullptr };
-    if (pay2) {
-        q = base + os_temp_bytes<K>(n, total_bits);
-        for (int i = 0; i < 2; i++) { t2[i] = (uint32_t*)q; q += align_up(n * sizeof(uint32_t)); }
-    }
-    if (!ctrl_cleared) {
-        const hipError_t e = hipMemsetAsync(base, 0, os_clear_bytes<K>(n, total_bits), s);
-        if (e != hipSuccess) return e;
-    }
-    if constexpr (pre0) {
-        os_tile_hist_kernel<<<(unsigned)blocks, 1024, 0, s>>>((const uint16_t*)kin, (uint32_t)n, plan, table);
-        os_table_scan_kernel<<<(unsigned)((1 << plan.bits[0]) + (plan.passes > 1 ? (1 << plan.bits[1]) : 0)), 256, 0, s>>>(table, (uint32_t)blocks, plan, hist);
+    if constexpr (os_table_driven<K>()) {
+        uint32_t* table = behind_hist;
+        int shift = 0;
+        for (int p = 0; p < plan.passes; p++) {
+            const bool last = p == plan.passes - 1;
+            const K* ki = p == 0 ? kin : tk[(p - 1) & 1];
+            const uint32_t* vi = p == 0 ? vin : tv[(p - 1) & 1];
+            uint32_t* h = hist + (size_t)p * OS_RADIX;
+            os_tile_hist_kernel<<<(unsigned)blocks, 1024, 0, s>>>((const uint16_t*)ki, (uint32_t)n, shift, plan.bits[p], table);
+            os_table_scan_kernel<<<1u << plan.bits[p], 256, 0, s>>>(table, (uint32_t)blocks, h);
+            os_launch_pass<K, true>(plan.bits[p], (unsigned)blocks, s, ki, last ? kout : tk[p & 1], vi, last ? vout : tv[p & 1], (uint32_t)n,
+                                    shift, h, table, nullptr, last ? gather_src : nullptr, last ? gather_dst : nullptr);
+            shift += plan.bits[p];
+        }
+        return hipGetLastError();
     } else {
-        const size_t nvec16 = n * sizeof(K) / 16 + 1;
-        const unsigned hb = (unsigned)std::min<size_t>((nvec16 + OS_HIST_BLOCK * 4 - 1) / (OS_HIST_BLOCK * 4), 512);
-        os_hist_kernel<K><<<hb, OS_HIST_BLOCK, 0, s>>>(kin, n, plan, hist);
-    }
-    int shift = 0;
-    for (int p = 0; p < plan.passes; p++) {
-        const K* ki = p == 0 ? kin : tk[(p - 1) & 1];
-        const uint32_t* vi = p == 0 ? vin : tv[(p - 1) & 1];
-        K* ko = p == plan.passes - 1 ? kout : tk[p & 1];
-        uint32_t* vo = p == plan.passes - 1 ? vout : tv[p & 1];
-        const bool last = p == plan.passes - 1;
-        if constexpr (sizeof(K) == 4) {
-            if (pay2) {
+        uint32_t* status = behind_hist;
+        uint32_t* ticket = status + (size_t)plan.passes * blocks * OS_RADIX;
+        uint32_t* t2[2] = { nullptr, nullptr };
+        if (pay2) {
+            q = base + os_temp_bytes<K>(n, total_bits);
+            for (int i = 0; i < 2; i++) { t2[i] = (uint32_t*)q; q += align_up(n * sizeof(uint32_t)); }
+        }
+        if (!ctrl_cleared) {
+            const hipError_t e = hipMemsetAsync(base, 0, os_clear_bytes<K>(n, total_bits), s);
+            if (e != hipSuccess) return e;
+        }
+        if (!hist_done) os_hist_kernel<K><<<os_hist_blocks<K>(n), OS_HIST_BLOCK, 0, s>>>(kin, n, plan, hist);
+        int shift = 0;
+        for (int p = 0; p < plan.passes; p++) {
+            const K* ki = p == 0 ? kin : tk[(p - 1) & 1];
+            const uint32_t* vi = p == 0 ? vin : tv[(p - 1) & 1];
+            K* ko = p == plan.passes - 1 ? kout : tk[p & 1];
+            uint32_t* vo = p == plan.passes - 1 ? vout : tv[p & 1];
+            const bool last = p == plan.passes - 1;
+            if (pay2)
                 os_pass_kernel<K, 8, false, true><<<(unsigned)blocks, OsShape<K>::BLOCK, 0, s>>>(
                     ki, ko, vi, vo, (uint32_t)n, shift, hist + (size_t)p * OS_RADIX, status + (size_t)p * blocks * OS_RADIX, ticket + p,
                     gather_src, gather_dst, p == 0 ? nullptr : t2[(p - 1) & 1], last ? nullptr : t2[p & 1]);
-                shift += plan.bits[p];
-                continue;
-            }
-        }
-        if (pre0 && p == 0)
-            os_launch_pass<K, true>(plan.bits[p], (unsigned)blocks, s, ki, ko, vi, vo, (uint32_t)n, shift, hist, table, ticket,
-                                    last ? gather_src : nullptr, last ? gather_dst : nullptr);
-        else
-            os_launch_pass<K, false>(plan.bits[p], (unsigned)blocks, s, ki, ko, vi, vo, (uint32_t)n, shift, hist + (size_t)p * OS_RADIX,
-                                     status + (size_t)p * blocks * OS_RADIX, ticket + p, last ? gather_src : nullptr, last ? gather_dst : nullptr);
-        shift += plan.bits[p];
-    }
-    return hipGetLastError();
+            else
+                os_launch_pass<K, false>(plan.bits[p], (unsigned)blocks, s, ki, ko, vi, vo, (uint32_t)n, shift, hist + (size_t)p * OS_RADIX,
+                                         status + (size_t)p * blocks * OS_RADIX, ticket + p, last ? gather_src : nullptr, last ? gather_dst : nullptr);
+            shift += plan.bits[p];
+        }
+        return hipGetLastError();
+    }
 }
 
 #ifdef C3DGS_DIAG
@@ -468,12 +494,22 @@
 {
     return os_sort<uint32_t>(temp, temp_bytes, kin, kout, vin, vout, (size_t)R, end_bit, s, nullptr, nullptr, ctrl_cleared);
 }
+hipError_t onesweep_depth_hist_scan(void* temp, size_t temp_bytes, const uint32_t* keys, int P, int nb, uint32_t* base,
+                                    const uint32_t* sort_err, uint32_t* host_out, uint32_t host_seq, hipStream_t s)
+{
+    const size_t n = (size_t)P;
+    if (P <= 0 || n >= ((size_t)1 << 30) || os_temp_bytes<uint32_t>(n, 32) > temp_bytes) return hipErrorInvalidValue;
+    os_hist_scan_kernel<<<1u + os_hist_blocks<uint32_t>(n), OS_HIST_BLOCK, 0, s>>>(keys, n, os_plan(32), (uint32_t*)temp, nb, base,
+                                                                                  sort_err, host_out, host_seq);
+    return hipGetLastError();
+}
 hipError_t onesweep_depth_sort(void* temp, size_t temp_bytes, const uint32_t* kin, uint32_t* kout, const uint32_t* vin, uint32_t* vout,
-                               int P, const uint2* gather_src, uint2* gather_dst, hipStream_t s, bool ctrl_cleared, bool rects_fit_bytes)
+                               int P, const uint2* gather_src, uint2* gather_dst, hipStream_t s, bool ctrl_cleared, bool rects_fit_bytes,
+                               bool hist_done)
 {
     static const bool no_pay2 = []() { const char* e = std::getenv("C3DGS_DEPTH_SORT_GATHER"); return e && e[0] == '1'; }();
     return os_sort<uint32_t>(temp, temp_bytes, kin, kout, vin, vout, (size_t)P, 32, s, gather_src, gather_dst, ctrl_cleared,
-                             rects_fit_bytes && !no_pay2);
+                             rects_fit_bytes && !no_pay2, hist_done && ctrl_cleared);
 }
 hipError_t onesweep_tile_sort(void* temp, size_t temp_bytes, const uint16_t* kin, uint16_t* kout, const uint32_t* vin, uint32_t* vout,
                               int R, int end_bit, hipStream_t s, bool ctrl_cleared)
diff --git a/c3dgs_amd/csrc/scan_blocks.hpp b/c3dgs_amd/csrc/scan_blocks.hpp
--- /dev/null
+++ b/c3dgs_amd/csrc/scan_blocks.hpp
@@ -0,0 +1,68 @@
+#pragma once
+#include <hip/hip_runtime.h>
+#include <cstdint>
+
+namespace c3dgs {
+
+constexpr int SCAN_BLOCKS_THREADS = 1024;
+
+__device__ __forceinline__ void scan_blocks_body(int nb, uint32_t* __restrict__ base, const uint32_t* __restrict__ sort_err,
+                                                 uint32_t* __restrict__ host_out, uint32_t host_seq)
+{
+    __shared__ uint32_t s_w[2][16];
+    const int t = threadIdx.x, lane = t & 63, wave = t >> 6;
+    uint32_t carry = 0;
+    int buf = 0;
+    for (int c0 = 0; c0 < nb; c0 += 16384, buf ^= 1) {
+        const int i0 = c0 + t * 16;
+        uint32_t v[16];
+#pragma unroll
+        for (int q = 0; q < 4; q++) {
+            uint4 x = make_uint4(0u, 0u, 0u, 0u);
+            if (i0 + 4 * q + 3 < nb) x = reinterpret_cast<const uint4*>(base + i0)[q];
+            else {
+                if (i0 + 4 * q < nb) x.x = base[i0 + 4 * q];
+                if (i0 + 4 * q + 1 < nb) x.y = base[i0 + 4 * q + 1];
+                if (i0 + 4 * q + 2 < nb) x.z = base[i0 + 4 * q + 2];
+            }
+            v[4 * q] = x.x; v[4 * q + 1] = x.y; v[4 * q + 2] = x.z; v[4 * q + 3] = x.w;
+        }
+        uint32_t mine = 0;
+#pragma unroll
+        for (int q = 0; q < 16; q++) mine += v[q];
+        uint32_t incl = mine;
+#pragma unroll
+        for (int o = 1; o < 64; o <<= 1) { const uint32_t u = __shfl_up(incl, o); if (lane >= o) incl += u; }
+        if (lane == 63) s_w[buf][wave] = incl;
+        __syncthreads();
+        uint32_t off = carry, all = 0;
+#pragma unroll
+        for (int w = 0; w < 16; w++) { const uint32_t x = s_w[buf][w]; if (w < wave) off += x; all += x; }
+        uint32_t run = off + incl - mine;
+#pragma unroll
+        for (int q = 0; q < 16; q++) { const uint32_t x = v[q]; v[q] = run; run += x; }
+#pragma unroll
+        for (int q = 0; q < 4; q++) {
+            if (i0 + 4 * q + 3 < nb) reinterpret_cast<uint4*>(base + i0)[q] = make_uint4(v[4 * q], v[4 * q + 1], v[4 * q + 2], v[4 * q + 3]);
+            else {
+                if (i0 + 4 * q < nb) base[i0 + 4 * q] = v[4 * q];
+                if (i0 + 4 * q + 1 < nb) base[i0 + 4 * q + 1] = v[4 * q + 1];
+                if (i0 + 4 * q + 2 < nb) base[i0 + 4 * q + 2] = v[4 * q + 2];
+            }
+        }
+        carry += all;
+    }
+    __syncthreads();
+    if (t == 0) {
+        base[nb] = carry;
+        const uint32_t err = sort_err ? *sort_err : 0u;
+        if (sort_err) base[nb + 1] = err;
+        if (host_out) {
+            __hip_atomic_store(host_out, carry, __ATOMIC_RELAXED, __HIP_MEMORY_SCOPE_SYSTEM);
+            __hip_atomic_store(host_out + 1, err, __ATOMIC_RELAXED, __HIP_MEMORY_SCOPE_SYSTEM);
+            __hip_atomic_store(host_out + 2, host_seq, __ATOMIC_RELEASE, __HIP_MEMORY_SCOPE_SYSTEM);
+        }
+    }
+}
+
+}
```

After: 635.3 views/s, median of 6. 2.0% higher.
